# wolny/pytorch-3dunet

Hardware: AMD Instinct MI355X
Metric: volumetric patches/sec (fwd+bwd), UNet3D f_maps=32 patch 64x128x128 (higher is better)
Workload: dtype f32

## Files before the change

include/u3d.h:

```cpp
#ifndef U3D_H
#define U3D_H

#include <stddef.h>
#include <stdint.h>

#ifdef __cplusplus
extern "C" {
#endif

#define U3D_VERSION 128

#define U3D_OK 0
#define U3D_EINVAL (-1)
#define U3D_EHIP (-2)
#define U3D_EARCH (-3)
#define U3D_EWORKSPACE (-4)

typedef void* u3d_stream_t;

typedef struct {
    const float* p0;
    const float* p1;
    const int32_t* zmap;
    const int32_t* ymap;
    const int32_t* xmap;
    const float* affine;
    int32_t C0, C1;
    int32_t D1, H1, W1;
} u3d_src_t;

int u3d_version(void);
const char* u3d_last_error(void);
int u3d_check_device(int device);
int u3d_set_tuning(int key, int value);
int u3d_set_profile_buffer(void* device_buffer, size_t bytes);
int u3d_debug_stream_pass(int device, u3d_stream_t stream, float* buf, long long n, int blocks, int passes, double min_seconds);
int u3d_debug_mfma_f32_rate(int device, u3d_stream_t stream, float* sink, int iters, int mode, double* flop_out);

size_t u3d_packed_weight_floats(int Cin, int Cout, int mode);
int u3d_pack_weights(int device, u3d_stream_t stream, const float* w, int Cout, int Cin, int mode, float* packed);
typedef struct {
    const float* w;
    float* packed;
    int64_t first;
    int32_t Cout, Cin, mode, cin_stride;
} u3d_pack_desc_t;
int u3d_pack_weights_batch(int device, u3d_stream_t stream, const u3d_pack_desc_t* descs_device, int n,
                           int64_t total_floats);
long long u3d_pack_weights_cells_blocks(const float* w, int Cin, int Cout, int mode, int cin_stride);
int u3d_pack_weights_batch_cells(int device, u3d_stream_t stream, const u3d_pack_desc_t* descs_device, int n, long long total_blocks);

int u3d_conv3d(int device, u3d_stream_t stream, const u3d_src_t* src, const float* packed_w, float* out,
               int N, int D, int H, int W, int Cout, int relu, double* out_stats, const u3d_src_t* gx,
               double* gstats);

int u3d_conv3d_residual(int device, u3d_stream_t stream, const u3d_src_t* src, const float* packed_w, float* out,
                        int N, int D, int H, int W, int Cout, int relu, double* out_stats, const float* residual);

long long u3d_conv3d_workspace_floats(int N, int D, int H, int W, int Cin, int Cout);
int u3d_conv3d_ex(int device, u3d_stream_t stream, const u3d_src_t* src, const float* packed_w, float* out, int N,
                  int D, int H, int W, int Cout, int relu, double* out_stats, const u3d_src_t* gx, double* gstats,
                  const float* residual, float* workspace, long long workspace_floats);

int u3d_conv3d_ex_reps(int device, u3d_stream_t stream, const u3d_src_t* src, const float* packed_w, float* out, int N,
                       int D, int H, int W, int Cout, int relu, double* out_stats, const u3d_src_t* gx, double* gstats,
                       const float* residual, float* workspace, long long workspace_floats, int stat_reps);

long long u3d_subpixel_packed_floats(int C1, int Cout);
long long u3d_subpixel_dgrad_packed_floats(int Cout, int C1);
int u3d_pack_subpixel_dgrad_weights(int device, u3d_stream_t stream, const float* w, int Cout, int Cin_total, int c_off,
                                    int C1, float* packed);
int u3d_subpixel_conv_dgrad(int device, u3d_stream_t stream, const float* dz, const float* packed, const float* x_low,
                            float* dlow, double* gstats, int N, int D1, int H1, int W1, int C1, int Cout);
int u3d_subpixel_conv_dgrad_reps(int device, u3d_stream_t stream, const float* dz, const float* packed, const float* x_low, float* dlow,
                                 double* gstats, int N, int D1, int H1, int W1, int C1, int Cout, int reps);
int u3d_pack_subpixel_weights(int device, u3d_stream_t stream, const float* w, int Cout, int Cin_total, int c_off, int C1,
                              float* packed);
long long u3d_subpixel_fwd_workspace_floats(int N, int D1, int H1, int W1, int C1, int Cout);
int u3d_subpixel_conv_fwd(int device, u3d_stream_t stream, const float* low, const float* affine,
                          long long affine_sample_stride, const float* packed, float* out, int N, int D1, int H1, int W1,
                          int C1, int Cout, float* workspace, long long workspace_floats);

size_t u3d_wgrad_workspace_floats(int N, int D, int H, int W, int Cin, int Cout);
int u3d_conv3d_wgrad(int device, u3d_stream_t stream, const u3d_src_t* src, const float* dz, float* dw, int N,
                     int D, int H, int W, int Cout, float* workspace, size_t workspace_floats);

int u3d_conv3d_variant(int N, int D, int H, int W, int Cin, int Cout, int src_kind, int has_workspace);
int u3d_conv3d_wgrad_variant(int N, int D, int H, int W, int Cin, int Cout, int src_kind);

int u3d_conv3d_wgrad_strided(int device, u3d_stream_t stream, const u3d_src_t* src, const float* dz, float* dw,
                             int dw_cin_stride, int N, int D, int H, int W, int Cout, float* workspace,
                             size_t workspace_floats);

typedef struct u3d_gn_bwd_job {
    const double* gstats_lo;
    const double* gstats_hi;
    const float* mean_rstd;
    const float* gamma;
    float* dgamma;
    float* dbeta;
    float* coef;
    float* coef_hi;
    double count;
    int32_t C0, C1, N, G;
    float hi_scale;
    int32_t reps_lo;
    int32_t reps_hi;
    int32_t reserved;
} u3d_gn_bwd_job_t;
int u3d_conv3d_wgrad_job_supported(int N, int C, int G);
int u3d_conv3d_wgrad_job(int device, u3d_stream_t stream, const u3d_src_t* src, const float* dz, float* dw, int dw_cin_stride,
                         int N, int D, int H, int W, int Cout, float* workspace, size_t workspace_floats,
                         const u3d_gn_bwd_job_t* job);

long long u3d_subpixel_wgrad_workspace_floats(int N, int D1, int H1, int W1, int C1, int Cout);
int u3d_subpixel_conv_wgrad(int device, u3d_stream_t stream, const float* low, const float* affine,
                            long long affine_sample_stride, const float* dz, float* dw, int dw_cin_stride, int N, int D1,
                            int H1, int W1, int C1, int Cout, float* workspace, long long workspace_floats);

int u3d_subpixel_conv_fwd_win(int device, u3d_stream_t stream, const float* low, const float* affine, long long affine_sample_stride,
                              const float* packed, float* out, int N, int D1, int H1, int W1, int C1, int Cout, const int* win);
int u3d_subpixel_conv_dgrad_win(int device, u3d_stream_t stream, const float* dz, const float* packed, const float* x_low, float* dlow,
                                double* gstats, int N, int D1, int H1, int W1, int C1, int Cout, const int* win);
int u3d_subpixel_conv_wgrad_win(int device, u3d_stream_t stream, const float* low, const float* affine, long long affine_sample_stride,
                                const float* dz, float* dw, int dw_cin_stride, int N, int D1, int H1, int W1, int C1, int Cout,
                                float* workspace, long long workspace_floats, const int* win);
int u3d_conv3d_box(int device, u3d_stream_t stream, const u3d_src_t* src, const float* packed_w, float* out, int N, int D, int H, int W,
                   int Cout, const int* out_box, const int* in_mask);
int u3d_conv3d_wgrad_box(int device, u3d_stream_t stream, const u3d_src_t* src, const float* dz, float* dw, int N, int D, int H, int W,
                         int Cout, float* workspace, size_t workspace_floats, const int* box);
int u3d_gn_bwd_apply_children(int device, u3d_stream_t stream, const float* dlow, const float* x, const float* coef, int Ctot, int coff,
                              int N, int D1, int H1, int W1, int C, int ez, int ey, int ex, int relu_mask, float* out);
int u3d_chan_stats_children(int device, u3d_stream_t stream, const float* x_low, int N, int D1, int H1, int W1, int C, int ez, int ey,
                            int ex, double* stats);
int u3d_nearest_childsum_add(int device, u3d_stream_t stream, const float* dv, const float* x_low, float* dlow, double* gstats, int N,
                             int D, int H, int W, int D1, int H1, int W1, int C, const int32_t* zlo, const int32_t* ylo,
                             const int32_t* xlo, int cz, int cy, int cx);

int u3d_conv3d_small_cin_fwd(int device, u3d_stream_t stream, const float* x, const float* affine, const float* w,
                             float* out, int N, int D, int H, int W, int Cin, int Cout, int relu, double* out_stats);
int u3d_conv3d_small_cin_fwd_reps(int device, u3d_stream_t stream, const float* x, const float* affine, const float* w, float* out, int N,
                                  int D, int H, int W, int Cin, int Cout, int relu, double* out_stats, int reps);
size_t u3d_small_cin_bwd_workspace_floats(int N, int D, int H, int W, int Cin, int Cout);
int u3d_conv3d_small_cin_bwd(int device, u3d_stream_t stream, const float* x, const float* affine, const float* dz,
                             const float* w, float* dw, double* gstats, int N, int D, int H, int W, int Cin, int Cout,
                             float* workspace, size_t workspace_floats);

int u3d_conv3d_naive(int device, u3d_stream_t stream, const u3d_src_t* src, const float* w, float* out, int N,
                     int D, int H, int W, int Cin, int Cout, int relu, int flip);
// ... 313 lines not shown
```

pytorch-3dunet_amd/csrc/u3d_conv.hip:

```cpp
#include <type_traits>
#include <utility>

#include "u3d_common.h"
#include "u3d_gn.h"
#include "u3d_subpix.h"

int g_u3d_tune[24] = {0};

namespace cv {
constexpr int TZ = 4, TY = 8, TX = 8;
constexpr int HZ = TZ + 2, HY = TY + 2, HX = TX + 2;
constexpr int CC = 16;
constexpr int CS = 16;
constexpr int RS = HX * CS + 4;
constexpr int PS = HY * RS;
constexpr int TILE_FLOATS = HZ * PS + 4;
constexpr int CNT_OFF = 2 * TILE_FLOATS;
constexpr int RED_OFF = CNT_OFF + 16;
constexpr int LDS_FLOATS = RED_OFF + 4 * 3 * 32 * 2;
constexpr int NITEMS = HZ * HY * HX * (CC / 4);
constexpr int NIT = (NITEMS + 255) / 256;
constexpr int NSTEP = 27 * (CC / 8);
constexpr int NSTEP_PAIRY = 36 * (CC / 8);
constexpr int NSTEP_N16 = 27;
constexpr int ST0 = 30;
constexpr int ISTORE = 5;
constexpr int PACK_PAD = 5;
static_assert(2 * (NIT - 1) < ST0 - 8 && ST0 + NIT <= NSTEP, "prefetch schedule must fit the k-loop");
}

struct ConvParams {
    u3d_src_t src;
    u3d_src_t gx;
    const float* wp;
    float* out;
    double* out_stats;
    double* gstats;
    const float* res;
    int N, D, H, W, Cout;
    int nchunks, ncb, ntot;
    int tz, ty, tx;
    int relu, vec, has_gx, ovec;
    int total;
    int gx_x2;
    int stagger;
    int stat_reps;
    int zfast;
    int ksplit, cps;
    long long part_stride;
    long long* dbg;
    int oz0, oy0, ox0, oz1, oy1, ox1;
    int mz, my, mx;
};

#define U3D_DBG_STAMP(slot)                                                   \
    do {                                                                      \
        if constexpr (DBG) {                                                  \
            if (l == 0) dbgw[slot] = (long long)__builtin_readcyclecounter(); \
        }                                                                     \
    } while (0)

__device__ __forceinline__ void u3d_flag_signal(int* c, int lane) {
    asm volatile("" ::: "memory");
    if (lane == 0) __hip_atomic_fetch_add(c, 1, __ATOMIC_RELAXED, __HIP_MEMORY_SCOPE_WORKGROUP);
    asm volatile("" ::: "memory");
}
__device__ __forceinline__ void u3d_flag_wait(int* c, int target) {
    while (__hip_atomic_load(c, __ATOMIC_RELAXED, __HIP_MEMORY_SCOPE_WORKGROUP) < target) __builtin_amdgcn_s_sleep(2);
    asm volatile("" ::: "memory");
}

template <int NT, bool VEC, bool DBG = false, int ABL = 0>
__global__ __launch_bounds__(256, 2) void conv3d_mfma_kernel(const ConvParams p) {
    using namespace cv;
    constexpr int RB = NT == 1 ? 6 : 3;
    extern __shared__ __attribute__((aligned(16))) float lds[];
    int* cnt = reinterpret_cast<int*>(lds + CNT_OFF);
    const int t = threadIdx.x;
    const int l = t & 63, w = t >> 6, m = l & 31, h = l >> 5;
    __builtin_amdgcn_s_setprio(3);
    long long* dbgw = nullptr;
    if constexpr (DBG) {
        dbgw = p.dbg + ((size_t)blockIdx.x * 4 + w) * 24;
        if (l == 0) {
            dbgw[0] = blockIdx.x;
            dbgw[1] = __builtin_amdgcn_s_getreg((31 << 11) | 4);
            dbgw[2] = __builtin_amdgcn_s_getreg((31 << 11) | 20);
            dbgw[7] = p.nchunks;
        }
    }
    U3D_DBG_STAMP(3);
    if (t < 16) cnt[t] = 0;
    __syncthreads();

    int logical = u3d_xcd_remap(blockIdx.x, gridDim.x);
    int ch0 = 0, nch = p.nchunks;
    float* const outp = p.out + (size_t)(p.ksplit > 1 ? logical % p.ksplit : 0) * p.part_stride;
    if (p.ksplit > 1) {
        ch0 = (logical % p.ksplit) * p.cps;
        nch = min(p.cps, p.nchunks - ch0);
        logical /= p.ksplit;
    }
    const int cb = logical % p.ncb;
    int tile = logical / p.ncb;
    const int txi = tile % p.tx;
    tile /= p.tx;
    const int tyi = tile % p.ty;
    tile /= p.ty;
    const int tzi = tile % p.tz;
    const int n = tile / p.tz;
    const int z0 = p.oz0 + tzi * TZ, y0 = p.oy0 + tyi * TY, x0 = p.ox0 + txi * TX;
    const int D = p.D, H = p.H, W = p.W;
    const int Ctot = p.src.C0 + p.src.C1;
    const bool slab_mask = (p.mz | p.my | p.mx) != 0;

    int ldsoff[NIT], gv0[NIT], gv1[NIT];
    const int q = t & 3;
#pragma unroll
    for (int it = 0; it < NIT; ++it) {
        const int item = t + 256 * it;
        const int vox = item >> 2;
        const bool in = item < NITEMS;
        const int hz = vox / (HY * HX);
        const int rem = vox - hz * (HY * HX);
        const int hy = rem / HX;
        const int hx = rem - hy * HX;
        ldsoff[it] = in ? hz * PS + hy * RS + hx * CS + 4 * q : HZ * PS;
        const int gz = z0 - 1 + hz, gy = y0 - 1 + hy, gxx = x0 - 1 + hx;
        bool ok = in && gz >= 0 && gz < D && gy >= 0 && gy < H && gxx >= 0 && gxx < W;
        if (slab_mask) ok = ok && ((p.mz && gz < p.mz) || (p.my && gy < p.my) || (p.mx && gxx < p.mx));
        gv0[it] = -1;
        gv1[it] = 0;
        if (ok) u3d_vox_index(p.src, n, gz, gy, gxx, D, H, W, gv0[it], gv1[it]);
    }

// ... 313 lines not shown
        if (arrived == 3) {
            for (int k = l; k < NT * 32; k += 64) {
                const int nt = k >> 5, mm = k & 31;
                float a = 0.f, b = 0.f;
#pragma unroll
                for (int ww = 0; ww < 4; ++ww) {
                    a += red[((ww * NT + nt) * 32 + mm) * 2 + 0];
                    b += red[((ww * NT + nt) * 32 + mm) * 2 + 1];
                }
                const int co = (cb * NT + nt) * 32 + mm;
                if (co < p.Cout) {
                    double* dst = (want_stats ? p.out_stats : p.gstats) + ((size_t)n * p.Cout + co) * 2;
                    u3d_atomic_add_f64(dst, (double)a);
                    u3d_atomic_add_f64(dst + 1, (double)b);
                }
            }
        }
    }
    U3D_DBG_STAMP(6);
}

struct SplitKParams {
    const float* part;
    long long stride;
    float* out;
    const float* res;
    double* stats;
    u3d_src_t gx;
    int ksplit, relu, want_g, V, D, H, W, C;
};

__global__ __launch_bounds__(256) void splitk_reduce_kernel(const SplitKParams p) {
    __shared__ double red[256 * 4 * 2];
    const int Q = p.C >> 2, per = blockDim.x / Q;
    const int t = threadIdx.x, cq = t % Q, vl = t / Q, n = blockIdx.y;
    for (int k = t; k < Q * 8; k += blockDim.x) red[k] = 0.0;
    __syncthreads();
    f32x4 s1 = {0.f, 0.f, 0.f, 0.f}, s2 = {0.f, 0.f, 0.f, 0.f};
    const bool xfrom0 = 4 * cq < p.gx.C0;
    for (int v = blockIdx.x * per + vl; v < p.V; v += gridDim.x * per) {
        const size_t off = ((size_t)n * p.V + v) * p.C + 4 * cq;
        f32x4 a = *reinterpret_cast<const f32x4*>(p.part + off);
        for (int k = 1; k < p.ksplit; ++k) a += *reinterpret_cast<const f32x4*>(p.part + (size_t)k * p.stride + off);
        if (p.res) a += *reinterpret_cast<const f32x4*>(p.res + off);
        if (p.relu) {
#pragma unroll
            for (int e = 0; e < 4; ++e) a[e] = fmaxf(a[e], 0.f);
        }
        *reinterpret_cast<f32x4*>(p.out + off) = a;
        if (p.stats) {
            s1 += a;
            if (p.want_g) {
                const int x = v % p.W, y = (v / p.W) % p.H, z = v / (p.W * p.H);
                int v0, v1;
                u3d_vox_index(p.gx, n, z, y, x, p.D, p.H, p.W, v0, v1);
                const f32x4 xv = xfrom0 ? *reinterpret_cast<const f32x4*>(p.gx.p0 + (size_t)v0 * p.gx.C0 + 4 * cq)
                                        : *reinterpret_cast<const f32x4*>(p.gx.p1 + (size_t)v1 * p.gx.C1 + (4 * cq - p.gx.C0));
                s2 += a * xv;
            } else {
                s2 += a * a;
            }
        }
    }
    if (p.stats) {
#pragma unroll
        for (int e = 0; e < 4; ++e) {
            __hip_atomic_fetch_add(&red[(cq * 4 + e) * 2], (double)s1[e], __ATOMIC_RELAXED, __HIP_MEMORY_SCOPE_WORKGROUP);
            __hip_atomic_fetch_add(&red[(cq * 4 + e) * 2 + 1], (double)s2[e], __ATOMIC_RELAXED, __HIP_MEMORY_SCOPE_WORKGROUP);
        }
        __syncthreads();
        for (int k = t; k < p.C * 2; k += blockDim.x) u3d_atomic_add_f64(&p.stats[(size_t)n * p.C * 2 + k], red[k]);
    }
}

template <int B, int... I, class F>
__device__ __forceinline__ void u3d_for_rows_impl(std::integer_sequence<int, I...>, F&& f) {
    (f(std::integral_constant<int, B + I>{}), ...);
}
template <int B, int E, class F>
__device__ __forceinline__ void u3d_for_rows(F&& f) {
    if constexpr (E > B) u3d_for_rows_impl<B>(std::make_integer_sequence<int, E - B>{}, static_cast<F&&>(f));
}

template <int NT, bool VIRT, bool DBG = false, bool PAIRY = false, bool AFF = true, bool N16 = false, bool RAG = false>
__global__ __launch_bounds__(256, 2) void conv3d_mfma_reg_kernel(const ConvParams p) {
    using namespace cv;
    static_assert(!RAG || (!PAIRY && !DBG), "ragged tiles: standard and 16-column variants only");
    static_assert(!PAIRY || NT == 1, "the paired-y variant has a single N-tile");
    static_assert(!N16 || (NT == 1 && !PAIRY), "the 16-column variant has a single N-tile");
    constexpr int RB = NT == 1 ? 9 : 3;
    constexpr int MT = N16 ? 4 : (PAIRY ? 1 : 2);
    constexpr int RY = PAIRY ? 4 : 3;
    constexpr int NROWS = 3 * RY;
    constexpr int SPR = N16 ? 3 : 6;
    constexpr int NSTEPL = NROWS * SPR;
    constexpr int DBG_TILE = 1;
    extern __shared__ __attribute__((aligned(16))) float lds[];
    int* cnt = reinterpret_cast<int*>(lds + CNT_OFF);
    double* red = reinterpret_cast<double*>(lds + RED_OFF);
    static_assert((RED_OFF * 4) % 8 == 0 && 2 * 3 * 32 * 2 * 8 <= 4 * 3 * 32 * 2 * 4, "f64 statistics rows must fit");
    const int t = threadIdx.x;
    const int l = t & 63, w = __builtin_amdgcn_readfirstlane(t >> 6), m = l & 31, h = l >> 5;
    __builtin_amdgcn_s_setprio(3);
    long long* dbgw = nullptr;
    if constexpr (DBG) {
        dbgw = p.dbg + ((size_t)blockIdx.x * 4 + w) * 24;
        if (l == 0) {
            dbgw[0] = blockIdx.x;
            dbgw[1] = __builtin_amdgcn_s_getreg((31 << 11) | 4);
            dbgw[2] = __builtin_amdgcn_s_getreg((31 << 11) | 20);
            dbgw[7] = p.nchunks;
        }
    }
    U3D_DBG_STAMP(3);
    if (t < 16) cnt[t] = 0;
    for (int k = t; k < 2 * 3 * 32 * 2; k += 256) red[k] = 0.0;
    __syncthreads();

    const int D = p.D, H = p.H, W = p.W;
    const int Ctot = p.src.C0 + p.src.C1;
    const int G = gridDim.x;
    const int D1 = p.src.D1, H1 = p.src.H1, W1 = p.src.W1;

    struct Item {
        int cb, n, z0, y0, x0;
        int base0, base1;
        unsigned inv;
        bool border;
    };
    const int q = t & 3, tv = t >> 2;
    int rel0[NIT], rel1[VIRT ? NIT : 1], loff[NIT];
    unsigned fz0 = 0, fz1 = 0, fy0 = 0, fy1 = 0, fx0 = 0, fx1 = 0, fdead = 0;
    const int vz = RAG && D % TZ ? D % TZ : TZ, vy = RAG && H % TY ? H % TY : TY, vx = RAG && W % TX ? W % TX : TX;
#pragma unroll
    for (int it = 0; it < NIT; ++it) {
        const int vox = tv + 64 * it;
        const bool in = vox < HZ * HY * HX;
        const int hz = vox / (HY * HX);
        const int rem = vox - hz * (HY * HX);
        const int hy = rem / HX;
        const int hx = rem - hy * HX;
        rel0[it] = in ? (hz * H + hy) * W + hx : 0;
        if constexpr (VIRT) rel1[it] = in ? (((hz - 1) >> 1) * H1 + ((hy - 1) >> 1)) * W1 + ((hx - 1) >> 1) : 0;
        loff[it] = in ? hz * PS + hy * RS + hx * CS + 4 * q : HZ * PS;
        fz0 |= (in && hz == 0 ? 1u : 0u) << it;
        fz1 |= (in && hz > vz ? 1u : 0u) << it;
        fy0 |= (in && hy == 0 ? 1u : 0u) << it;
        fy1 |= (in && hy > vy ? 1u : 0u) << it;
        fx0 |= (in && hx == 0 ? 1u : 0u) << it;
        fx1 |= (in && hx > vx ? 1u : 0u) << it;
        fdead |= (in ? 0u : 1u) << it;
    }
    struct Digits {
        int cb, xi, yi, zi, n;
    };
    const bool zfast = p.zfast != 0;
    const int r1 = zfast ? p.tz : p.tx, r3 = zfast ? p.tx : p.tz;
    auto decode = [&](int idx) {
        Digits d;
        d.cb = idx % p.ncb;
        int tile = idx / p.ncb;
        d.xi = tile % r1;
        tile /= r1;
        d.yi = tile % p.ty;
        tile /= p.ty;
        d.zi = tile % r3;
        d.n = tile / r3;
        return d;
    };
    const Digits dG = decode(G);
    auto advance = [&](const Digits& a) {
        Digits r;
        int c;
        r.cb = a.cb + dG.cb;
        c = r.cb >= p.ncb ? 1 : 0;
        r.cb -= c ? p.ncb : 0;
        r.xi = a.xi + dG.xi + c;
        c = r.xi >= r1 ? 1 : 0;
        r.xi -= c ? r1 : 0;
        r.yi = a.yi + dG.yi + c;
        c = r.yi >= p.ty ? 1 : 0;
        r.yi -= c ? p.ty : 0;
        r.zi = a.zi + dG.zi + c;
        c = r.zi >= r3 ? 1 : 0;
        r.zi -= c ? r3 : 0;
        r.n = a.n + dG.n + c;
        return r;
    };
    auto item_of = [&](const Digits& d) {
        Item c;
        c.cb = d.cb;
        c.x0 = (zfast ? d.zi : d.xi) * TX;
        c.y0 = d.yi * TY;
        c.z0 = (zfast ? d.xi : d.zi) * TZ;
        c.n = d.n;
        c.base0 = ((c.n * D + c.z0 - 1) * H + c.y0 - 1) * W + c.x0 - 1;
        c.base1 = VIRT ? ((c.n * D1 + (c.z0 >> 1)) * H1 + (c.y0 >> 1)) * W1 + (c.x0 >> 1) : 0;
        const bool bz0 = c.z0 == 0, bz1 = c.z0 + TZ >= D, by0 = c.y0 == 0, by1 = c.y0 + TY >= H, bx0 = c.x0 == 0,
                   bx1 = c.x0 + TX >= W;
        c.border = bz0 || bz1 || by0 || by1 || bx0 || bx1;
        c.inv = fdead | (bz0 ? fz0 : 0u) | (bz1 ? fz1 : 0u) | (by0 ? fy0 : 0u) | (by1 ? fy1 : 0u) | (bx0 ? fx0 : 0u) |
                (bx1 ? fx1 : 0u);
        return c;
    };
    int wi = u3d_xcd_remap(blockIdx.x, G);
    Digits dT = decode(wi);
    Item T = item_of(dT);

    constexpr bool ZEROC = NT < 3 && !N16;
    f32x16 acc[N16 ? 1 : MT][NT];
    f32x4 acc16[N16 ? MT : 1];
    if constexpr (N16) {
#pragma unroll
        for (int mt = 0; mt < MT; ++mt) acc16[mt] = f32x4{0.f, 0.f, 0.f, 0.f};
    } else if constexpr (!ZEROC) {
#pragma unroll
        for (int mt = 0; mt < MT; ++mt)
#pragma unroll
            for (int nt = 0; nt < NT; ++nt)
#pragma unroll
                for (int r = 0; r < 16; ++r) acc[mt][nt][r] = 0.f;
    }

    const int v16 = l & 15, kq = l >> 4;
    const int abase = N16 ? w * PS + 2 * (v16 >> 3) * RS + (v16 & 7) * CS + 4 * kq
                          : w * PS + (m >> 3) * (PAIRY ? 2 : 1) * RS + (m & 7) * CS + 4 * h;
    auto mrow = [](int mt) { return N16 ? (mt >> 1) * 4 + (mt & 1) : 4 * mt; };

    const f32x4* wimg = reinterpret_cast<const f32x4*>(p.wp);
    const f32x4* wq = wimg + (size_t)T.cb * NT * 64;
    const int wstep = p.ntot * 64;
    f32x4 bq[RB][NT];
#pragma unroll
    for (int k = 0; k < RB - 1; ++k)
#pragma unroll
        for (int nt = 0; nt < NT; ++nt) bq[k][nt] = wq[(size_t)k * wstep + nt * 64 + l];

    struct ChunkSrc {
        const float* base;
        int Cs;
        bool cok, from0;
        const float* ap;
        f32x4 lo, hi;
    };
    auto chunk_src = [&](int ch, int n, bool live) {
        ChunkSrc c;
        const int cq = ch * CC + 4 * q;
        c.cok = live && cq < Ctot;
        c.from0 = !VIRT || cq < p.src.C0;
        c.base = !c.cok ? p.src.p0 : (c.from0 ? p.src.p0 + cq : p.src.p1 + (cq - p.src.C0));
        c.Cs = (c.from0 || !c.cok) ? p.src.C0 : p.src.C1;
        c.ap = p.src.affine ? p.src.affine + ((size_t)n * Ctot + (c.cok ? cq : 0)) * 2 : nullptr;
        c.lo = f32x4{1.f, 0.f, 1.f, 0.f};
        c.hi = f32x4{1.f, 0.f, 1.f, 0.f};
        return c;
    };
    auto load_affine_rows = [&](ChunkSrc& c) {
        if constexpr (AFF) {
            if (c.ap) {
                c.lo = *reinterpret_cast<const f32x4*>(c.ap);
                c.hi = *reinterpret_cast<const f32x4*>(c.ap + 4);
            }
        }
    };
    auto halo_load = [&](const ChunkSrc& c, const Item& S, int it, bool masked) {
        int idx = c.from0 ? S.base0 + rel0[it] : S.base1 + rel1[VIRT ? it : 0];
        if (masked) idx = (c.cok && ((S.inv >> it) & 1u) == 0) ? idx : 0;
        return *reinterpret_cast<const f32x4*>(c.base + (size_t)idx * c.Cs);
    };
    auto halo_store = [&](float* buf, const ChunkSrc& c, const Item& S, int it, f32x4 raw, bool masked) {
        f32x4 val = raw;
        if constexpr (AFF)
            val = f32x4{fmaf(raw[0], c.lo[0], c.lo[1]), fmaf(raw[1], c.lo[2], c.lo[3]), fmaf(raw[2], c.hi[0], c.hi[1]),
                        fmaf(raw[3], c.hi[2], c.hi[3])};
        if (masked) {
            const bool ok = c.cok && ((S.inv >> it) & 1u) == 0;
#pragma unroll
            for (int e = 0; e < 4; ++e) val[e] = ok ? val[e] : 0.f;
        }
        *reinterpret_cast<f32x4*>(&buf[loff[it]]) = val;
    };
    const bool want_stats = p.out_stats != nullptr;
    const bool want_g = p.gstats != nullptr;
    auto flush_stats = [&](int n, int cb) {
        if (!(want_stats || want_g)) return;
        const int par = n & 1;
        int arrived = 0;
        asm volatile("" ::: "memory");
        if (l == 0) arrived = __hip_atomic_fetch_add(&cnt[5 + par], 1, __ATOMIC_RELAXED, __HIP_MEMORY_SCOPE_WORKGROUP);
        arrived = __builtin_amdgcn_readfirstlane(arrived);
        asm volatile("" ::: "memory");
        if ((arrived & 3) != 3) return;
        const int rep = p.stat_reps > 1 ? (int)(blockIdx.x % (unsigned)p.stat_reps) : 0;
        for (int k = l; k < NT * 32; k += 64) {
            double* r = &red[(par * NT * 32 + k) * 2];
            const double a = r[0], b = r[1];
            r[0] = 0.0;
            r[1] = 0.0;
            const int co = cb * NT * 32 + k;
            if (co < p.Cout) {
                double* dst = (want_stats ? p.out_stats : p.gstats) + ((size_t)rep * p.N * p.Cout + (size_t)n * p.Cout + co) * 2;
                u3d_atomic_add_f64(dst, a);
                u3d_atomic_add_f64(dst + 1, b);
            }
        }
        asm volatile("" ::: "memory");
    };
    const bool dead_quads = (Ctot % CC) != 0;

    {
        ChunkSrc c0 = chunk_src(0, T.n, true);
        load_affine_rows(c0);
        const bool masked = T.border || dead_quads || fdead != 0;
        f32x4 v[NIT];
#pragma unroll
        for (int it = 0; it < NIT; ++it) v[it] = halo_load(c0, T, it, true);
#pragma unroll
        for (int it = 0; it < NIT; ++it) halo_store(lds, c0, T, it, v[it], true);
        (void)masked;
    }
    u3d_flag_signal(&cnt[0], l);

    if (p.stagger > 0 && (int)blockIdx.x >= (G + 1) / 2) {
        for (int i = 0; i < p.stagger; ++i) __builtin_amdgcn_s_sleep(16);
    }

    int gch = 0;
    int ntiles = 0;
    constexpr bool CARRY = NT == 1;
    f32x4 sq1 = {0.f, 0.f, 0.f, 0.f}, sq2 = {0.f, 0.f, 0.f, 0.f};
    auto quad_sum = [](float v) {
        v += __builtin_bit_cast(float, __builtin_amdgcn_mov_dpp(__builtin_bit_cast(int, v), 0xB1, 0xF, 0xF, true));
        v += __builtin_bit_cast(float, __builtin_amdgcn_mov_dpp(__builtin_bit_cast(int, v), 0x4E, 0xF, 0xF, true));
        return v;
    };
    auto stat_reduce = [&](const f32x4& a1, const f32x4& a2, int n_, int nt_, int c0) {
#pragma unroll
        for (int e = 0; e < 4; ++e) {
            const float a = quad_sum(a1[e]), b2 = quad_sum(a2[e]);
            if ((l & 3) == 0) {
                double* r = &red[(((n_ & 1) * NT + nt_) * 32 + c0 + e) * 2];
                __hip_atomic_fetch_add(r, (double)a, __ATOMIC_RELAXED, __HIP_MEMORY_SCOPE_WORKGROUP);
                __hip_atomic_fetch_add(r + 1, (double)b2, __ATOMIC_RELAXED, __HIP_MEMORY_SCOPE_WORKGROUP);
            }
        }
    };
    while (true) {
        const int nwi = wi + G;
        const bool has_next_tile = nwi < p.total;
        const Digits dTN = has_next_tile ? advance(dT) : dT;
        const Item TN = item_of(dTN);
        const f32x4* wqn = wimg + (size_t)TN.cb * NT * 64;

        for (int ch = 0; ch < p.nchunks; ++ch, ++gch) {
            const bool last = ch + 1 == p.nchunks;
            const bool has_next = !last || has_next_tile;
            const int b = gch & 1;
            const float* cur = lds + b * TILE_FLOATS;
            float* nxt = lds + (b ^ 1) * TILE_FLOATS;
            const int nch_ = last ? 0 : ch + 1;
            const Item S = last ? TN : T;
            ChunkSrc cn = chunk_src(nch_, S.n, has_next);
            const bool masked = S.border || !has_next || (dead_quads && nch_ + 1 == p.nchunks);
            f32x4 v[NIT];
            u3d_flag_wait(&cnt[b], 4 * (gch / 2 + 1));
            __builtin_amdgcn_s_setprio(0);
            if (ntiles == DBG_TILE && ch < 7) U3D_DBG_STAMP(8 + 2 * ch);
            if (ntiles == DBG_TILE + 1 && ch == 0) U3D_DBG_STAMP(23);

            f32x4 aq[2][MT];
#pragma unroll
            for (int mt = 0; mt < MT; ++mt) aq[0][mt] = *reinterpret_cast<const f32x4*>(&cur[abase + mrow(mt) * RS]);
            const f32x4* wch0 = wq + (size_t)(ch * NSTEPL + RB - 1) * wstep;
            enum { ROW_PLAIN = 0, ROW_LOAD = 1, ROW_AFFINE = 2, ROW_STORE = 3, ROW_LAST = 4, ROW_LOAD_FIRST = 5 };
            auto row_body = [&](auto kind_c, auto row_c) __attribute__((always_inline)) {
                constexpr int KIND = decltype(kind_c)::value;
                constexpr int row = decltype(row_c)::value;
                const int rz = row / RY, ry = row - RY * rz;
                const float* arow = cur + abase + rz * PS + ry * RS;
                const int nrow = row + 1;
                const float* anext = cur + abase + (nrow / RY) * PS + (nrow % RY) * RS;
                const bool do_store = KIND == ROW_STORE && has_next;
                if constexpr (KIND == ROW_AFFINE) load_affine_rows(cn);
                if constexpr (KIND == ROW_STORE) {
                    if (do_store) u3d_flag_wait(&cnt[2 + (b ^ 1)], 4 * ((gch + 1) / 2));
                }
#pragma unroll
                for (int s6 = 0; s6 < SPR; ++s6) {
                    constexpr int STORES_PER_STEP = (NIT + SPR - 2) / (SPR - 1);
                    {
                        const f32x4* wsrc = wch0 + (size_t)(row * SPR + s6) * wstep;
                        if (row * SPR + s6 + RB - 1 >= NSTEPL && last) wsrc = wqn + (size_t)(row * SPR + s6 + RB - 1 - NSTEPL) * wstep;
#pragma unroll
                        for (int nt = 0; nt < NT; ++nt) bq[(row * SPR + s6 + RB - 1) % RB][nt] = wsrc[nt * 64 + l];
                    }
                    if constexpr (KIND == ROW_LOAD || KIND == ROW_LOAD_FIRST) {
                        if (s6 == 0) {
                            if (masked) {
#pragma unroll
                                for (int it = 0; it < NIT; ++it) v[it] = halo_load(cn, S, it, true);
                            } else {
#pragma unroll
                                for (int it = 0; it < NIT; ++it) v[it] = halo_load(cn, S, it, false);
                            }
                        }
                    }
                    __builtin_amdgcn_sched_barrier(0);
#pragma unroll
                    for (int j = 0; j < 2; ++j) {
                        if constexpr (N16) {
#pragma unroll
                            for (int mt = 0; mt < MT; ++mt)
                                acc16[mt] = __builtin_amdgcn_mfma_f32_16x16x4f32(bq[(row * SPR + s6) % RB][0][j], aq[(row * SPR + s6) & 1][mt][j], acc16[mt], 0, 0, 0);
                        } else {
#pragma unroll
                            for (int nt = 0; nt < NT; ++nt) {
#pragma unroll
                                for (int mt = 0; mt < MT; ++mt) {
                                    if (KIND == ROW_LOAD_FIRST && s6 == 0 && j == 0) {
                                        const f32x16 zero = {0.f, 0.f, 0.f, 0.f, 0.f, 0.f, 0.f, 0.f, 0.f, 0.f, 0.f, 0.f, 0.f, 0.f, 0.f, 0.f};
                                        acc[mt][nt] = __builtin_amdgcn_mfma_f32_32x32x2f32(aq[0][mt][0], bq[0][nt][0], zero, 0, 0, 0);
                                    } else {
                                        acc[mt][nt] = __builtin_amdgcn_mfma_f32_32x32x2f32(aq[(row * SPR + s6) & 1][mt][j], bq[(row * SPR + s6) % RB][nt][j], acc[mt][nt], 0, 0, 0);
                                    }
                                }
                            }
                        }
                    }
                    __builtin_amdgcn_sched_barrier(0);
                    if (s6 < SPR - 1) {
                        const int aoff = N16 ? (s6 + 1) * CS : ((s6 + 1) >> 1) * CS + 8 * ((s6 + 1) & 1);
#pragma unroll
                        for (int mt = 0; mt < MT; ++mt) aq[(row * SPR + s6 + 1) & 1][mt] = *reinterpret_cast<const f32x4*>(&arow[mrow(mt) * RS + aoff]);
                    } else if constexpr (KIND != ROW_LAST) {
#pragma unroll
                        for (int mt = 0; mt < MT; ++mt) aq[(row * SPR + s6 + 1) & 1][mt] = *reinterpret_cast<const f32x4*>(&anext[mrow(mt) * RS]);
                    }
                    if constexpr (KIND == ROW_STORE) {
                        if (do_store && s6 * STORES_PER_STEP < NIT) {
#pragma unroll
                            for (int k = 0; k < STORES_PER_STEP; ++k) {
                                const int it = s6 * STORES_PER_STEP + k;
                                if (it < NIT) {
                                    if (masked)
                                        halo_store(nxt, cn, S, it, v[it], true);
                                    else
                                        halo_store(nxt, cn, S, it, v[it], false);
                                }
                            }
                            if ((s6 + 1) * STORES_PER_STEP >= NIT) u3d_flag_signal(&cnt[b ^ 1], l);
                        }
                    }
                    __builtin_amdgcn_sched_barrier(0);
#pragma unroll
                    for (int j = 2; j < 4; ++j) {
                        if constexpr (N16) {
#pragma unroll
                            for (int mt = 0; mt < MT; ++mt)
                                acc16[mt] = __builtin_amdgcn_mfma_f32_16x16x4f32(bq[(row * SPR + s6) % RB][0][j], aq[(row * SPR + s6) & 1][mt][j], acc16[mt], 0, 0, 0);
                        } else {
#pragma unroll
                            for (int nt = 0; nt < NT; ++nt) {
#pragma unroll
                                for (int mt = 0; mt < MT; ++mt)
                                    acc[mt][nt] = __builtin_amdgcn_mfma_f32_32x32x2f32(aq[(row * SPR + s6) & 1][mt][j], bq[(row * SPR + s6) % RB][nt][j], acc[mt][nt], 0, 0, 0);
                            }
                        }
                    }
                    __builtin_amdgcn_sched_barrier(0);
                }
            };
            static_assert(ISTORE - 1 > 1 && ISTORE + 1 < NROWS - 1, "row kinds must not collide");
            static_assert(NSTEPL % RB == 0, "B ring slots are indexed by the k-step within the chunk");
            using R0 = std::integral_constant<int, 0>;
            if (ZEROC && ch == 0)
                row_body(std::integral_constant<int, ROW_LOAD_FIRST>{}, R0{});
            else
                row_body(std::integral_constant<int, ROW_LOAD>{}, R0{});
            u3d_for_rows<1, ISTORE - 1>([&](auto r) { row_body(std::integral_constant<int, ROW_PLAIN>{}, r); });
            row_body(std::integral_constant<int, ROW_AFFINE>{}, std::integral_constant<int, ISTORE - 1>{});
            row_body(std::integral_constant<int, ROW_STORE>{}, std::integral_constant<int, ISTORE>{});
            u3d_for_rows<ISTORE + 1, NROWS - 1>([&](auto r) { row_body(std::integral_constant<int, ROW_PLAIN>{}, r); });
            row_body(std::integral_constant<int, ROW_LAST>{}, std::integral_constant<int, NROWS - 1>{});
            if (ntiles == DBG_TILE && ch < 7) U3D_DBG_STAMP(9 + 2 * ch);
            u3d_flag_signal(&cnt[2 + b], l);
        }
        __builtin_amdgcn_s_setprio(3);

        if (ntiles == DBG_TILE) U3D_DBG_STAMP(5);
        if constexpr (N16) {
            const int n = T.n;
            const int z = T.z0 + w;
            const int co = 4 * kq;
            const bool cok = co < p.Cout;
            const int vlane = ((n * D + z) * H + T.y0 + 2 * (v16 >> 3)) * W + T.x0 + (v16 & 7);
            float* orow = p.out + (size_t)vlane * p.Cout + co;
            const size_t rstep = (size_t)W * p.Cout;
            auto vin = [&](int mt) { return !RAG || (z < D && T.y0 + mrow(mt) + 2 * (v16 >> 3) < H && T.x0 + (v16 & 7) < W); };
            f32x4 xv[MT];
            if (want_g) {
                const bool from0 = co < p.gx.C0 || !cok;
#pragma unroll
                for (int mt = 0; mt < MT; ++mt) {
                    const int y = T.y0 + mrow(mt) + 2 * (v16 >> 3), x = T.x0 + (v16 & 7);
                    const int xi1 = ((n * p.gx.D1 + (z >> 1)) * p.gx.H1 + (y >> 1)) * p.gx.W1 + (x >> 1);
                    const float* xp = !(cok && vin(mt)) ? p.gx.p0
                                           : (from0 ? p.gx.p0 + (size_t)(vlane + mrow(mt) * W) * p.gx.C0 + co
                                                    : p.gx.p1 + (size_t)xi1 * p.gx.C1 + (co - p.gx.C0));
                    xv[mt] = *reinterpret_cast<const f32x4*>(xp);
                }
            } else if (p.res) {
#pragma unroll
                for (int mt = 0; mt < MT; ++mt)
                    xv[mt] = *reinterpret_cast<const f32x4*>(p.res + (vin(mt) ? (size_t)(vlane + mrow(mt) * W) * p.Cout + (cok ? co : 0) : (size_t)0));
            }
#pragma unroll
            for (int mt = 0; mt < MT; ++mt) {
                f32x4 val = acc16[mt];
                if (p.res) val += xv[mt];
                if (p.relu) {
#pragma unroll
                    for (int e = 0; e < 4; ++e) val[e] = fmaxf(val[e], 0.f);
                }
                if (cok && vin(mt)) *reinterpret_cast<f32x4*>(orow + mrow(mt) * rstep) = val;
                if (RAG || p.Cout % 16 != 0) {
#pragma unroll
                    for (int e = 0; e < 4; ++e) val[e] = (cok && vin(mt)) ? val[e] : 0.f;
                }
                sq1 += val;
                sq2 += want_g ? val * xv[mt] : val * val;
                acc16[mt] = f32x4{0.f, 0.f, 0.f, 0.f};
            }
        } else
        if (p.stagger != -1) {
            const int n = T.n, cb = T.cb;
            const int z = T.z0 + w;
            const int cq = (l >> 2) & 7, vl = (l & 3) + 4 * h;
            const bool odd = (l & 1) != 0, hi = (l & 2) != 0;
            auto xlane = [](float v, auto ctrl) {
                return __builtin_bit_cast(float, __builtin_amdgcn_mov_dpp(__builtin_bit_cast(int, v), decltype(ctrl)::value, 0xF, 0xF, true));
            };
            using X1 = std::integral_constant<int, 0xB1>;
            using X2 = std::integral_constant<int, 0x4E>;
            const int vrow = ((n * D + z) * H + T.y0) * W + T.x0 + vl;
            const int xrow = ((n * p.gx.D1 + (z >> 1)) * p.gx.H1 + (T.y0 >> 1)) * p.gx.W1 + ((T.x0 + vl) >> 1);
#pragma unroll
            for (int nt = 0; nt < NT; ++nt) {
                f32x4 q1 = {0.f, 0.f, 0.f, 0.f}, q2 = {0.f, 0.f, 0.f, 0.f};
                f32x4 tq[4 * MT];
#pragma unroll
                for (int mt = 0; mt < MT; ++mt)
#pragma unroll
                    for (int bi = 0; bi < 4; ++bi) {
                        const float a0 = acc[mt][nt][4 * bi + 0], a1 = acc[mt][nt][4 * bi + 1];
                        const float a2 = acc[mt][nt][4 * bi + 2], a3 = acc[mt][nt][4 * bi + 3];
                        const float t0 = xlane(a1, X1{}), t1 = xlane(a0, X1{}), t2 = xlane(a3, X1{}), t3 = xlane(a2, X1{});
                        const float c0 = odd ? t0 : a0, c1 = odd ? a1 : t1, c2 = odd ? t2 : a2, c3 = odd ? a3 : t3;
                        const float u0 = xlane(c2, X2{}), u2 = xlane(c0, X2{}), u1 = xlane(c3, X2{}), u3 = xlane(c1, X2{});
                        tq[4 * mt + bi] = f32x4{hi ? u0 : c0, hi ? u1 : c1, hi ? c2 : u2, hi ? c3 : u3};
                    }
                const int ysh = PAIRY ? (cq >> 2) : 0;
                const int co = PAIRY ? 4 * (cq & 3) : (cb * NT + nt) * 32 + 4 * cq;
// ... 793 lines not shown
            const int f = fq * (sp::NFRAG / PK_SUBQ) + (i >> 6), lane = i & 63;
            const int st = sp::frag_tab().st[f];
            const int kl = 8 * (st & 1) + 4 * (lane >> 5), nl = lane & 31;
            f32x4 v;
#pragma unroll
            for (int j = 0; j < 4; ++j) v[j] = sp::frag_value(row_of(nl, kl + j), f);
            out4[(((long long)ch * sp::NFRAG + f) * ntot + ntg) * 64 + lane] = v;
        }
    } else {
        for (int i = t; i < spd::NFRAG / PK_SUBQ * 64; i += 256) {
            const int f = fq * (spd::NFRAG / PK_SUBQ) + (i >> 6), lane = i & 63;
            const int kl = 8 * (f & 1) + 4 * (lane >> 5), nl = lane & 31;
            f32x4 v;
#pragma unroll
            for (int j = 0; j < 4; ++j) v[j] = spd::frag_value(row_of(nl, kl + j), f);
            out4[(((long long)ch * spd::NFRAG + f) * ntot + ntg) * 64 + lane] = v;
        }
    }
}

__global__ void conv3d_naive_kernel(const u3d_src_t src, const float* __restrict__ w, float* __restrict__ out,
                                    int N, int D, int H, int W, int Cin, int Cout, int relu, int flip) {
    const long long total = (long long)N * D * H * W * Cout;
    for (long long idx = (long long)blockIdx.x * blockDim.x + threadIdx.x; idx < total;
         idx += (long long)gridDim.x * blockDim.x) {
        const int co = (int)(idx % Cout);
        long long v = idx / Cout;
        const int x = (int)(v % W);
        v /= W;
        const int y = (int)(v % H);
        v /= H;
        const int z = (int)(v % D);
        const int n = (int)(v / D);
        float sum = 0.f;
        for (int tap = 0; tap < 27; ++tap) {
            const int zz = z + tap / 9 - 1, yy = y + (tap / 3) % 3 - 1, xx = x + tap % 3 - 1;
            if (zz < 0 || zz >= D || yy < 0 || yy >= H || xx < 0 || xx >= W) continue;
            int v0, v1;
            u3d_vox_index(src, n, zz, yy, xx, D, H, W, v0, v1);
            for (int c = 0; c < Cin; ++c) {
                float g = u3d_load_elem(src, v0, v1, c);
                if (src.affine) {
                    const float* ab = src.affine + ((size_t)n * Cin + c) * 2;
                    g = g * ab[0] + ab[1];
                }
                const float wt = flip ? w[((size_t)c * Cout + co) * 27 + (26 - tap)] : w[((size_t)co * Cin + c) * 27 + tap];
                sum += g * wt;
            }
        }
        if (relu) sum = fmaxf(sum, 0.f);
        out[idx] = sum;
    }
}

static inline int cdiv(int a, int b) { return (a + b - 1) / b; }

static bool src_vec_ok(const u3d_src_t* s) {
    if (s->C0 % 4 != 0 || s->C1 % 4 != 0) return false;
    if (((uintptr_t)s->p0 & 15) != 0) return false;
    if (s->C1 > 0 && ((uintptr_t)s->p1 & 15) != 0) return false;
    if (s->affine && ((uintptr_t)s->affine & 15) != 0) return false;
    return true;
}

static int check_src(const u3d_src_t* s, const char* what) {
    U3D_REQUIRE(s != nullptr && s->p0 != nullptr && (s->C0 > 0 || s->C1 > 0) && s->C0 >= 0, "%s: null source", what);
    U3D_REQUIRE(s->C1 >= 0, "%s: negative C1", what);
    if (s->C1 > 0)
        U3D_REQUIRE(s->p1 && s->zmap && s->ymap && s->xmap && s->D1 > 0 && s->H1 > 0 && s->W1 > 0,
                    "%s: low-res source needs p1, index maps and dims", what);
    return 0;
}

static long long* g_u3d_prof_buf = nullptr;
static size_t g_u3d_prof_records = 0;

extern "C" int u3d_set_profile_buffer(void* device_buffer, size_t bytes) {
    g_u3d_prof_buf = static_cast<long long*>(device_buffer);
    g_u3d_prof_records = device_buffer ? bytes / (24 * sizeof(long long)) : 0;
    return 0;
}

extern "C" int u3d_set_tuning(int key, int value) {
    if (key < 0 || key >= 24) return u3d_set_err(U3D_EINVAL, "u3d_set_tuning: key out of range");
    g_u3d_tune[key] = value;
    return 0;
}

extern "C" size_t u3d_packed_weight_floats(int Cin, int Cout, int mode) {
    return (size_t)pack_total_floats(Cin, Cout, mode, nullptr, nullptr);
}

extern "C" int u3d_pack_weights(int device, u3d_stream_t stream, const float* w, int Cout, int Cin, int mode,
                                float* packed) {
    U3D_ENTER(device);
    U3D_REQUIRE(w && packed && Cout > 0 && Cin > 0 && (mode == 0 || mode == 1), "u3d_pack_weights: bad argument");
    int nchunks = 0, ntot = 0;
    const long long total = pack_total_floats(Cin, Cout, mode, &nchunks, &ntot);
    const int blocks = (int)((total + 255) / 256 > 4096 ? 4096 : (total + 255) / 256);
    hipLaunchKernelGGL(pack_weights_kernel, dim3(blocks), dim3(256), 0, (hipStream_t)stream, w, packed, Cout, Cin,
                       mode, nchunks, ntot, total);
    U3D_LAUNCH_CHECK();
    return 0;
}

extern "C" int u3d_pack_weights_batch(int device, u3d_stream_t stream, const u3d_pack_desc_t* descs_device, int n,
                                      int64_t total_floats) {
    U3D_ENTER(device);
    U3D_REQUIRE(descs_device && n > 0 && total_floats > 0, "u3d_pack_weights_batch: bad argument");
    U3D_REQUIRE(total_floats % 4 == 0, "u3d_pack_weights_batch: image sizes are multiples of 4 floats");
    long long blocks = (total_floats / 4 + 255) / 256;
    if (blocks > 8192) blocks = 8192;
    hipLaunchKernelGGL(pack_weights_batch_kernel, dim3((unsigned)blocks), dim3(256), 0, (hipStream_t)stream, descs_device, n,
                       (long long)total_floats);
    U3D_LAUNCH_CHECK();
    return 0;
}

extern "C" long long u3d_pack_weights_cells_blocks(const float* w, int Cin, int Cout, int mode, int cin_stride) {
    const int cs = cin_stride > 0 ? cin_stride : Cin;
    if (Cin <= 0 || Cout <= 0 || mode < 0 || mode > 3 || Cin % 4 != 0 || Cout % 4 != 0 || cs % 4 != 0 || ((uintptr_t)w & 15) != 0) return 0;
    return pack_cells_of(Cin, Cout, mode) + 1;
}

extern "C" int u3d_pack_weights_batch_cells(int device, u3d_stream_t stream, const u3d_pack_desc_t* descs_device, int n,
                                            long long total_blocks) {
    U3D_ENTER(device);
    U3D_REQUIRE(descs_device && n > 0 && total_blocks > 0 && total_blocks < 0x7fffffffLL, "u3d_pack_weights_batch_cells: bad argument");
    hipLaunchKernelGGL(pack_weights_cells_kernel, dim3((unsigned)total_blocks), dim3(256), 0, (hipStream_t)stream, descs_device, n);
    U3D_LAUNCH_CHECK();
    return 0;
}

static int device_cu_count(int device, int* out) {
    static int cached[64] = {0};
    if (device >= 0 && device < 64 && cached[device] > 0) {
        *out = cached[device];
        return 0;
    }
    int n = 0;
    U3D_HIP(hipDeviceGetAttribute(&n, hipDeviceAttributeMultiprocessorCount, device));
    if (n <= 0) n = 256;
    if (device >= 0 && device < 64) cached[device] = n;
    *out = n;
    return 0;
}

template <int NT>
static int conv_set_lds_nt() {
    const int bytes = cv::LDS_FLOATS * sizeof(float);
    U3D_HIP(hipFuncSetAttribute(reinterpret_cast<const void*>(conv3d_mfma_reg_kernel<NT, false, false>),
                                hipFuncAttributeMaxDynamicSharedMemorySize, bytes));
    U3D_HIP(hipFuncSetAttribute(reinterpret_cast<const void*>(conv3d_mfma_reg_kernel<NT, true, false>),
                                hipFuncAttributeMaxDynamicSharedMemorySize, bytes));
    U3D_HIP(hipFuncSetAttribute(reinterpret_cast<const void*>(conv3d_mfma_reg_kernel<NT, false, true>),
                                hipFuncAttributeMaxDynamicSharedMemorySize, bytes));
    U3D_HIP(hipFuncSetAttribute(reinterpret_cast<const void*>(conv3d_mfma_reg_kernel<NT, true, true>),
                                hipFuncAttributeMaxDynamicSharedMemorySize, bytes));
    U3D_HIP(hipFuncSetAttribute(reinterpret_cast<const void*>(conv3d_mfma_reg_kernel<NT, false, false, false, false>),
                                hipFuncAttributeMaxDynamicSharedMemorySize, bytes));
    U3D_HIP(hipFuncSetAttribute(reinterpret_cast<const void*>(conv3d_mfma_reg_kernel<NT, true, false, false, true, false, true>),
                                hipFuncAttributeMaxDynamicSharedMemorySize, bytes));
    U3D_HIP(hipFuncSetAttribute(reinterpret_cast<const void*>(conv3d_mfma_reg_kernel<NT, false, false, false, false, false, true>),
                                hipFuncAttributeMaxDynamicSharedMemorySize, bytes));
    U3D_HIP(hipFuncSetAttribute(reinterpret_cast<const void*>(conv3d_mfma_reg_kernel<NT, false, false, false, true, false, true>),
                                hipFuncAttributeMaxDynamicSharedMemorySize, bytes));
    if (NT == 1) {
        U3D_HIP(hipFuncSetAttribute(reinterpret_cast<const void*>(conv3d_mfma_reg_kernel<1, true, false, false, true, true, true>),
                                    hipFuncAttributeMaxDynamicSharedMemorySize, bytes));
        U3D_HIP(hipFuncSetAttribute(reinterpret_cast<const void*>(conv3d_mfma_reg_kernel<1, false, false, false, false, true, true>),
                                    hipFuncAttributeMaxDynamicSharedMemorySize, bytes));
        U3D_HIP(hipFuncSetAttribute(reinterpret_cast<const void*>(conv3d_mfma_reg_kernel<1, false, false, false, true, true, true>),
                                    hipFuncAttributeMaxDynamicSharedMemorySize, bytes));
        U3D_HIP(hipFuncSetAttribute(reinterpret_cast<const void*>(conv3d_mfma_reg_kernel<1, false, false, true, false>),
                                    hipFuncAttributeMaxDynamicSharedMemorySize, bytes));
        U3D_HIP(hipFuncSetAttribute(reinterpret_cast<const void*>(conv3d_mfma_reg_kernel<1, false, false, true>),
                                    hipFuncAttributeMaxDynamicSharedMemorySize, bytes));
        U3D_HIP(hipFuncSetAttribute(reinterpret_cast<const void*>(conv3d_mfma_reg_kernel<1, true, false, true>),
                                    hipFuncAttributeMaxDynamicSharedMemorySize, bytes));
        U3D_HIP(hipFuncSetAttribute(reinterpret_cast<const void*>(conv3d_mfma_reg_kernel<1, true, false, false, true, true>),
                                    hipFuncAttributeMaxDynamicSharedMemorySize, bytes));
        U3D_HIP(hipFuncSetAttribute(reinterpret_cast<const void*>(conv3d_mfma_reg_kernel<1, false, false, false, false, true>),
                                    hipFuncAttributeMaxDynamicSharedMemorySize, bytes));
        U3D_HIP(hipFuncSetAttribute(reinterpret_cast<const void*>(conv3d_mfma_reg_kernel<1, false, false, false, true, true>),
                                    hipFuncAttributeMaxDynamicSharedMemorySize, bytes));
    }
    U3D_HIP(hipFuncSetAttribute(reinterpret_cast<const void*>(conv3d_mfma_kernel<NT, true, false>),
                                hipFuncAttributeMaxDynamicSharedMemorySize, bytes));
    U3D_HIP(hipFuncSetAttribute(reinterpret_cast<const void*>(conv3d_mfma_kernel<NT, false, false>),
                                hipFuncAttributeMaxDynamicSharedMemorySize, bytes));
    U3D_HIP(hipFuncSetAttribute(reinterpret_cast<const void*>(conv3d_mfma_kernel<NT, true, true>),
                                hipFuncAttributeMaxDynamicSharedMemorySize, bytes));
    if (NT == 1) {
        U3D_HIP(hipFuncSetAttribute(reinterpret_cast<const void*>(conv3d_mfma_kernel<1, true, true, 1>),
                                    hipFuncAttributeMaxDynamicSharedMemorySize, bytes));
        U3D_HIP(hipFuncSetAttribute(reinterpret_cast<const void*>(conv3d_mfma_kernel<1, true, true, 2>),
                                    hipFuncAttributeMaxDynamicSharedMemorySize, bytes));
        U3D_HIP(hipFuncSetAttribute(reinterpret_cast<const void*>(conv3d_mfma_kernel<1, true, true, 3>),
                                    hipFuncAttributeMaxDynamicSharedMemorySize, bytes));
        U3D_HIP(hipFuncSetAttribute(reinterpret_cast<const void*>(conv3d_mfma_kernel<1, true, true, 7>),
                                    hipFuncAttributeMaxDynamicSharedMemorySize, bytes));
    }
    return 0;
}

static int conv_set_lds_once(int device) {
    static bool done[64] = {false};
    if (device >= 0 && device < 64 && done[device]) return 0;
    if (int e = conv_set_lds_nt<1>()) return e;
    if (int e = conv_set_lds_nt<2>()) return e;
    if (int e = conv_set_lds_nt<3>()) return e;
    if (device >= 0 && device < 64) done[device] = true;
    return 0;
}

static int conv3d_impl(int device, u3d_stream_t stream, const u3d_src_t* src, const float* packed_w, float* out, int N,
                       int D, int H, int W, int Cout, int relu, double* out_stats, const u3d_src_t* gx, double* gstats,
                       const float* residual, float* ws = nullptr, long long ws_floats = 0, const int* out_box = nullptr,
                       const int* in_mask = nullptr, int stat_reps = 1);

extern "C" int u3d_conv3d(int device, u3d_stream_t stream, const u3d_src_t* src, const float* packed_w, float* out,
                          int N, int D, int H, int W, int Cout, int relu, double* out_stats, const u3d_src_t* gx,
                          double* gstats) {
    return conv3d_impl(device, stream, src, packed_w, out, N, D, H, W, Cout, relu, out_stats, gx, gstats, nullptr);
}

extern "C" int u3d_conv3d_box(int device, u3d_stream_t stream, const u3d_src_t* src, const float* packed_w, float* out, int N, int D,
                              int H, int W, int Cout, const int* out_box, const int* in_mask) {
    return conv3d_impl(device, stream, src, packed_w, out, N, D, H, W, Cout, 0, nullptr, nullptr, nullptr, nullptr, nullptr, 0, out_box,
                       in_mask);
}

constexpr int SPLITK_MAX = 16;
static int g_u3d_ncu_seen = 256;
static int splitk_count(int ncu, long long ntiles, int ntot, int nchunks, int* cps_out) {
    long long ks = (2ll * ncu) / (ntiles * ntot);
    if (ks > nchunks) ks = nchunks;
    if (ks > SPLITK_MAX) ks = SPLITK_MAX;
    int cps = nchunks, ksplit = 1;
    if (ks >= 2) {
        cps = (nchunks + (int)ks - 1) / (int)ks;
        ksplit = (nchunks + cps - 1) / cps;
    }
    if (cps_out) *cps_out = cps;
    return ksplit;
}

static bool splitk_shape(int N, int D, int H, int W, int Cin, int Cout) {
    const long long items = (long long)N * cdiv(D, cv::TZ) * cdiv(H, cv::TY) * cdiv(W, cv::TX) * cdiv(Cout, 32);
    return Cin > 16 && Cout % 4 == 0 && Cout <= 1024 && items < 256;
}

extern "C" long long u3d_conv3d_workspace_floats(int N, int D, int H, int W, int Cin, int Cout) {
    if (N <= 0 || D <= 0 || H <= 0 || W <= 0 || Cin <= 0 || Cout <= 0 || !splitk_shape(N, D, H, W, Cin, Cout)) return 0;
    const int ks = cdiv(Cin, 16) < SPLITK_MAX ? cdiv(Cin, 16) : SPLITK_MAX;
    return (long long)ks * N * D * H * W * Cout;
}

extern "C" int u3d_conv3d_ex(int device, u3d_stream_t stream, const u3d_src_t* src, const float* packed_w, float* out,
                             int N, int D, int H, int W, int Cout, int relu, double* out_stats, const u3d_src_t* gx,
                             double* gstats, const float* residual, float* workspace, long long workspace_floats) {
    U3D_REQUIRE(!(residual && gx), "u3d_conv3d_ex: residual and gx are mutually exclusive");
    return conv3d_impl(device, stream, src, packed_w, out, N, D, H, W, Cout, relu, out_stats, gx, gstats, residual,
                       workspace, workspace_floats);
}

extern "C" int u3d_conv3d_ex_reps(int device, u3d_stream_t stream, const u3d_src_t* src, const float* packed_w, float* out,
                                  int N, int D, int H, int W, int Cout, int relu, double* out_stats, const u3d_src_t* gx,
                                  double* gstats, const float* residual, float* workspace, long long workspace_floats, int stat_reps) {
    U3D_REQUIRE(!(residual && gx), "u3d_conv3d_ex_reps: residual and gx are mutually exclusive");
    return conv3d_impl(device, stream, src, packed_w, out, N, D, H, W, Cout, relu, out_stats, gx, gstats, residual,
                       workspace, workspace_floats, nullptr, nullptr, stat_reps);
}

extern "C" int u3d_conv3d_residual(int device, u3d_stream_t stream, const u3d_src_t* src, const float* packed_w,
                                   float* out, int N, int D, int H, int W, int Cout, int relu, double* out_stats,
                                   const float* residual) {
    if (residual == nullptr) return u3d_set_err(U3D_EINVAL, "u3d_conv3d_residual: residual is NULL");
    return conv3d_impl(device, stream, src, packed_w, out, N, D, H, W, Cout, relu, out_stats, nullptr, nullptr, residual);
}

static int conv3d_impl(int device, u3d_stream_t stream, const u3d_src_t* src, const float* packed_w, float* out, int N,
                       int D, int H, int W, int Cout, int relu, double* out_stats, const u3d_src_t* gx, double* gstats,
                       const float* residual, float* ws, long long ws_floats, const int* out_box, const int* in_mask, int stat_reps) {
    U3D_ENTER(device);
    if (int e = check_src(src, "u3d_conv3d")) return e;
    U3D_REQUIRE(stat_reps >= 1 && stat_reps <= 64, "u3d_conv3d: stat_reps must be 1 .. 64");
    U3D_REQUIRE(packed_w && out && N > 0 && D > 0 && H > 0 && W > 0 && Cout > 0, "u3d_conv3d: bad argument");
    U3D_REQUIRE((long long)N * D * H * W < (1ll << 31), "u3d_conv3d: N*D*H*W must be < 2^31");
    U3D_REQUIRE(!(out_stats && gstats), "u3d_conv3d: out_stats and gstats are mutually exclusive");
    U3D_REQUIRE((gstats == nullptr) == (gx == nullptr), "u3d_conv3d: gx and gstats go together");
    U3D_REQUIRE(((uintptr_t)packed_w & 15) == 0, "u3d_conv3d: packed weights must be 16-byte aligned");
    ConvParams p;
    p.src = *src;
    if (gx) {
        if (int e = check_src(gx, "u3d_conv3d(gx)")) return e;
        U3D_REQUIRE(gx->C0 + gx->C1 == Cout, "u3d_conv3d: gx must have Cout channels");
        p.gx = *gx;
    } else {
        p.gx = *src;
    }
    p.has_gx = gx != nullptr;
    p.wp = packed_w;
    p.out = out;
    p.out_stats = out_stats;
    p.gstats = gstats;
    p.res = residual;
    p.N = N, p.D = D, p.H = H, p.W = W, p.Cout = Cout;
    const int Cin = src->C0 + src->C1;
    p.nchunks = cdiv(Cin, 16);
    p.ntot = cdiv(Cout, 32);
    p.tz = cdiv(D, cv::TZ), p.ty = cdiv(H, cv::TY), p.tx = cdiv(W, cv::TX);
    p.oz0 = p.oy0 = p.ox0 = 0, p.oz1 = D, p.oy1 = H, p.ox1 = W;
    p.mz = p.my = p.mx = 0;
    const bool boxed = out_box != nullptr || in_mask != nullptr;
    if (out_box) {
        U3D_REQUIRE(out_box[0] >= 0 && out_box[1] >= 0 && out_box[2] >= 0 && out_box[3] <= D && out_box[4] <= H && out_box[5] <= W &&
                        out_box[0] < out_box[3] && out_box[1] < out_box[4] && out_box[2] < out_box[5],
                    "u3d_conv3d_box: output box outside the volume or empty");
        p.oz0 = out_box[0], p.oy0 = out_box[1], p.ox0 = out_box[2], p.oz1 = out_box[3], p.oy1 = out_box[4], p.ox1 = out_box[5];
        p.tz = cdiv(p.oz1 - p.oz0, cv::TZ), p.ty = cdiv(p.oy1 - p.oy0, cv::TY), p.tx = cdiv(p.ox1 - p.ox0, cv::TX);
    }
    if (in_mask) p.mz = in_mask[0], p.my = in_mask[1], p.mx = in_mask[2];
    p.relu = relu;
    p.vec = src_vec_ok(src) ? 1 : 0;
    p.ovec = (Cout % 4 == 0 && ((uintptr_t)out & 15) == 0 && (!gx || src_vec_ok(gx)) &&
              (!residual || ((uintptr_t)residual & 15) == 0)) ? 1 : 0;
    const long long ntiles = (long long)N * p.tz * p.ty * p.tx;
    int nt = 1;
    if (p.ntot % 3 == 0 && ntiles * (p.ntot / 3) >= 512) nt = 3;
    else if (p.ntot % 2 == 0 && ntiles * (p.ntot / 2) >= 512) nt = 2;
    if (g_u3d_tune[0] >= 1 && g_u3d_tune[0] <= 3 && p.ntot % g_u3d_tune[0] == 0) nt = g_u3d_tune[0];
    p.ncb = p.ntot / nt;
    const long long nblk = ntiles * p.ncb;
    U3D_REQUIRE(nblk < (1ll << 31), "u3d_conv3d: grid too large");
    const size_t shmem = cv::LDS_FLOATS * sizeof(float);
    if (int e = conv_set_lds_once(device)) return e;
    hipStream_t st = (hipStream_t)stream;
    p.ksplit = 1, p.cps = p.nchunks, p.part_stride = 0;
    if (!boxed && ws && p.vec && p.ovec && ((uintptr_t)ws & 15) == 0 && splitk_shape(N, D, H, W, Cin, Cout) && g_u3d_tune[7] != 2) {
        int ncu = 0;
        if (int e = device_cu_count(device, &ncu)) return e;
        g_u3d_ncu_seen = ncu;
        const long long items = ntiles * p.ntot, out_elems = (long long)N * D * H * W * Cout;
        p.ksplit = splitk_count(ncu, ntiles, p.ntot, p.nchunks, &p.cps);
        if (p.ksplit >= 2 && (long long)p.ksplit * out_elems <= ws_floats) {
            p.ncb = p.ntot;
            p.part_stride = out_elems;
            p.out = ws;
            p.out_stats = nullptr, p.gstats = nullptr, p.res = nullptr, p.relu = 0, p.has_gx = 0, p.dbg = nullptr;
            const dim3 kgrid((unsigned)(items * p.ksplit)), kblock(256);
            hipLaunchKernelGGL((conv3d_mfma_kernel<1, true>), kgrid, kblock, shmem, st, p);
            U3D_LAUNCH_CHECK();
            SplitKParams r;
            r.part = ws, r.stride = out_elems, r.out = out, r.res = residual;
            r.stats = out_stats ? out_stats : gstats;
            r.gx = gx ? *gx : *src;
            r.ksplit = p.ksplit, r.relu = relu, r.want_g = gstats != nullptr;
            r.V = D * H * W, r.D = D, r.H = H, r.W = W, r.C = Cout;
            const int Q = Cout / 4, per = 256 / Q;
            int gxb = cdiv(r.V, per * 4);
            const int cap = 256 / N > 1 ? 256 / N : 1;
            if (gxb > cap) gxb = cap;
            hipLaunchKernelGGL(splitk_reduce_kernel, dim3((unsigned)gxb, (unsigned)N), dim3((unsigned)(Q * per)), 0, st, r);
            U3D_LAUNCH_CHECK();
            return 0;
        }
        p.ksplit = 1, p.cps = p.nchunks;
    }
    auto plain_or_x2 = [&](const u3d_src_t& s_) {
        return s_.C1 == 0 || (D == 2 * s_.D1 && H == 2 * s_.H1 && W == 2 * s_.W1);
    };
    const bool ragged = D % cv::TZ != 0 || H % cv::TY != 0 || W % cv::TX != 0;
    const bool reg = p.vec && p.ovec && plain_or_x2(p.src) && (!gx || plain_or_x2(p.gx)) && g_u3d_tune[3] == 0 ||
                     (g_u3d_tune[3] == 2 && !ragged && p.vec && p.ovec && plain_or_x2(p.src) && (!gx || plain_or_x2(p.gx)));
    if (reg && !boxed) {
        p.total = (int)nblk;
        p.gx_x2 = (gx && p.gx.C1 > 0) ? 1 : 0;
        p.stagger = g_u3d_tune[5];
        p.stat_reps = stat_reps;
        p.zfast = g_u3d_tune[14] == 1 ? 0 : 1;
        int ncu = 0;
        if (int e = device_cu_count(device, &ncu)) return e;
        long long slots = (g_u3d_tune[6] == 1 ? 1ll : 2ll) * ncu;
        if (g_u3d_tune[12] > 0 && g_u3d_tune[12] < slots / 2) slots -= g_u3d_tune[12];
        if (slots >= nblk)
            slots = nblk;
        else if (slots > p.ncb)
            slots -= slots % p.ncb;
        const dim3 rgrid((unsigned)slots), rblock(256);
        const bool virt = p.src.C1 > 0;
        const bool noaff = p.src.affine == nullptr && g_u3d_tune[7] == 0;
        p.dbg = (!ragged && g_u3d_prof_buf && (size_t)slots * 4 <= g_u3d_prof_records) ? g_u3d_prof_buf : nullptr;
        if (ragged) {
            if (Cout <= 16 && nt == 1 && p.ntot == 1) {
                p.wp = packed_w + ((size_t)p.nchunks * cv::NSTEP + cv::PACK_PAD) * 256 + ((size_t)p.nchunks * cv::NSTEP_PAIRY + cv::PACK_PAD) * 256;
                if (virt)
                    hipLaunchKernelGGL((conv3d_mfma_reg_kernel<1, true, false, false, true, true, true>), rgrid, rblock, shmem, st, p);
                else if (noaff)
                    hipLaunchKernelGGL((conv3d_mfma_reg_kernel<1, false, false, false, false, true, true>), rgrid, rblock, shmem, st, p);
                else
                    hipLaunchKernelGGL((conv3d_mfma_reg_kernel<1, false, false, false, true, true, true>), rgrid, rblock, shmem, st, p);
                U3D_LAUNCH_CHECK();
                return 0;
            }
#define U3D_RAG_LAUNCH(NT_)                                                                                                        \
    do {                                                                                                                           \
        if (virt)                                                                                                                  \
            hipLaunchKernelGGL((conv3d_mfma_reg_kernel<NT_, true, false, false, true, false, true>), rgrid, rblock, shmem, st, p);  \
        else if (noaff)                                                                                                            \
            hipLaunchKernelGGL((conv3d_mfma_reg_kernel<NT_, false, false, false, false, false, true>), rgrid, rblock, shmem, st, p); \
        else                                                                                                                       \
            hipLaunchKernelGGL((conv3d_mfma_reg_kernel<NT_, false, false, false, true, false, true>), rgrid, rblock, shmem, st, p); \
    } while (0)
            if (nt == 3)
                U3D_RAG_LAUNCH(3);
            else if (nt == 2)
                U3D_RAG_LAUNCH(2);
            else
                U3D_RAG_LAUNCH(1);
#undef U3D_RAG_LAUNCH
            U3D_LAUNCH_CHECK();
            return 0;
        }
        if (Cout <= 16 && nt == 1 && p.ntot == 1 && !p.dbg && g_u3d_tune[4] != 1) {
            const size_t std_floats = ((size_t)p.nchunks * cv::NSTEP + cv::PACK_PAD) * 256;
            if (g_u3d_tune[4] == 2) {
                p.wp = packed_w + std_floats;
                if (virt)
                    hipLaunchKernelGGL((conv3d_mfma_reg_kernel<1, true, false, true>), rgrid, rblock, shmem, st, p);
                else if (noaff)
                    hipLaunchKernelGGL((conv3d_mfma_reg_kernel<1, false, false, true, false>), rgrid, rblock, shmem, st, p);
                else
                    hipLaunchKernelGGL((conv3d_mfma_reg_kernel<1, false, false, true>), rgrid, rblock, shmem, st, p);
            } else {
                p.wp = packed_w + std_floats + ((size_t)p.nchunks * cv::NSTEP_PAIRY + cv::PACK_PAD) * 256;
                if (virt)
                    hipLaunchKernelGGL((conv3d_mfma_reg_kernel<1, true, false, false, true, true>), rgrid, rblock, shmem, st, p);
                else if (noaff)
                    hipLaunchKernelGGL((conv3d_mfma_reg_kernel<1, false, false, false, false, true>), rgrid, rblock, shmem, st, p);
                else
                    hipLaunchKernelGGL((conv3d_mfma_reg_kernel<1, false, false, false, true, true>), rgrid, rblock, shmem, st, p);
            }
            U3D_LAUNCH_CHECK();
            return 0;
        }
#define U3D_REG_LAUNCH(NT_)                                                                                \
    do {                                                                                                   \
        if (p.dbg && virt)                                                                                 \
            hipLaunchKernelGGL((conv3d_mfma_reg_kernel<NT_, true, true>), rgrid, rblock, shmem, st, p);    \
        else if (p.dbg)                                                                                    \
            hipLaunchKernelGGL((conv3d_mfma_reg_kernel<NT_, false, true>), rgrid, rblock, shmem, st, p);   \
        else if (virt)                                                                                     \
            hipLaunchKernelGGL((conv3d_mfma_reg_kernel<NT_, true, false>), rgrid, rblock, shmem, st, p);   \
        else if (noaff)                                                                                    \
            hipLaunchKernelGGL((conv3d_mfma_reg_kernel<NT_, false, false, false, false>), rgrid, rblock,   \
                               shmem, st, p);                                                              \
        else                                                                                               \
            hipLaunchKernelGGL((conv3d_mfma_reg_kernel<NT_, false, false>), rgrid, rblock, shmem, st, p);  \
    } while (0)
        if (nt == 3)
            U3D_REG_LAUNCH(3);
        else if (nt == 2)
            U3D_REG_LAUNCH(2);
        else
            U3D_REG_LAUNCH(1);
#undef U3D_REG_LAUNCH
        U3D_LAUNCH_CHECK();
        return 0;
    }
    const bool vec = p.vec != 0;
    const dim3 grid((unsigned)nblk), block(256);
    p.dbg = (vec && g_u3d_prof_buf && (size_t)nblk * 4 <= g_u3d_prof_records) ? g_u3d_prof_buf : nullptr;
#define U3D_CONV_LAUNCH(NT_)                                                                     \
    do {                                                                                         \
        if (p.dbg && NT_ == 1 && g_u3d_tune[2] == 1)                                             \
            hipLaunchKernelGGL((conv3d_mfma_kernel<1, true, true, 1>), grid, block, shmem, st, p); \
        else if (p.dbg && NT_ == 1 && g_u3d_tune[2] == 2)                                        \
            hipLaunchKernelGGL((conv3d_mfma_kernel<1, true, true, 2>), grid, block, shmem, st, p); \
        else if (p.dbg && NT_ == 1 && g_u3d_tune[2] == 3)                                        \
            hipLaunchKernelGGL((conv3d_mfma_kernel<1, true, true, 3>), grid, block, shmem, st, p); \
        else if (p.dbg && NT_ == 1 && g_u3d_tune[2] == 7)                                        \
            hipLaunchKernelGGL((conv3d_mfma_kernel<1, true, true, 7>), grid, block, shmem, st, p); \
        else if (p.dbg)                                                                          \
            hipLaunchKernelGGL((conv3d_mfma_kernel<NT_, true, true>), grid, block, shmem, st, p); \
        else if (vec)                                                                            \
            hipLaunchKernelGGL((conv3d_mfma_kernel<NT_, true>), grid, block, shmem, st, p);      \
        else                                                                                     \
            hipLaunchKernelGGL((conv3d_mfma_kernel<NT_, false>), grid, block, shmem, st, p);     \
    } while (0)
    if (nt == 3)
        U3D_CONV_LAUNCH(3);
    else if (nt == 2)
        U3D_CONV_LAUNCH(2);
    else
        U3D_CONV_LAUNCH(1);
#undef U3D_CONV_LAUNCH
    U3D_LAUNCH_CHECK();
    return 0;
}

static void wgrad_plan(int N, int D, int H, int W, int Cin, int Cout, WgradParams& p) {
    p.nchunks = cdiv(Cin, 32);
    p.nkb = cdiv(Cout, 32);
    p.tz = cdiv(D, wg::TZ), p.ty = cdiv(H, wg::TY), p.tx = cdiv(W, wg::TX);
    p.ntiles = N * p.tz * p.ty * p.tx;
    const int pairs = p.nchunks * p.nkb;
    const int ncu = 256;
    long long best_cost = -1;
    int best_S = 1;
    for (int rounds = 1; rounds <= 8; ++rounds) {
        int S = (rounds * ncu) / pairs;
        if (S < 1) S = 1;
        if (S > p.ntiles) S = p.ntiles;
        const int tps = cdiv(p.ntiles, S);
        S = cdiv(p.ntiles, tps);
        const long long cost = (long long)cdiv(S * pairs, ncu) * (tps + 2);
        if (best_cost < 0 || cost < best_cost) {
            best_cost = cost;
            best_S = S;
        }
    }
    if (g_u3d_tune[1] > 0) best_S = g_u3d_tune[1] > p.ntiles ? p.ntiles : g_u3d_tune[1];
    p.tps = cdiv(p.ntiles, best_S);
    p.S = cdiv(p.ntiles, p.tps);
}

extern "C" size_t u3d_wgrad_workspace_floats(int N, int D, int H, int W, int Cin, int Cout) {
    WgradParams p;
    wgrad_plan(N, D, H, W, Cin, Cout, p);
    return (size_t)p.S * p.nchunks * p.nkb * 27 * 1024;
}

static int wgrad_set_lds_once(int device) {
    static bool done[64] = {false};
    if (device >= 0 && device < 64 && done[device]) return 0;
    U3D_HIP(hipFuncSetAttribute(reinterpret_cast<const void*>(conv3d_wgrad_kernel<true, true>),
                                hipFuncAttributeMaxDynamicSharedMemorySize, (wg::LDS_FLOATS + wg::MAX_MAP_INTS) * sizeof(float)));
    U3D_HIP(hipFuncSetAttribute(reinterpret_cast<const void*>(conv3d_wgrad_kernel<true, true, true>),
                                hipFuncAttributeMaxDynamicSharedMemorySize, (wg::LDS_FLOATS + wg::MAX_MAP_INTS) * sizeof(float)));
    U3D_HIP(hipFuncSetAttribute(reinterpret_cast<const void*>(conv3d_wgrad_kernel<true>),
                                hipFuncAttributeMaxDynamicSharedMemorySize, (wg::LDS_FLOATS + wg::MAX_MAP_INTS) * sizeof(float)));
    U3D_HIP(hipFuncSetAttribute(reinterpret_cast<const void*>(conv3d_wgrad_kernel<false>),
                                hipFuncAttributeMaxDynamicSharedMemorySize, (wg::LDS_FLOATS + wg::MAX_MAP_INTS) * sizeof(float)));
    if (device >= 0 && device < 64) done[device] = true;
    return 0;
}

static int conv3d_wgrad_impl(int device, u3d_stream_t stream, const u3d_src_t* src, const float* dz, float* dw, int cstride,
                             int N, int D, int H, int W, int Cout, float* workspace, size_t workspace_floats, const int* box = nullptr,
                             const u3d_gn_bwd_job_t* job = nullptr);

extern "C" int u3d_conv3d_wgrad_box(int device, u3d_stream_t stream, const u3d_src_t* src, const float* dz, float* dw, int N, int D,
// ... 135 lines not shown
```

pytorch-3dunet_amd/csrc/u3d_gn.h:

```cpp
#pragma once
#include "u3d_common.h"

__device__ __forceinline__ double u3d_sum_replicas(const double* __restrict__ p, size_t stride, int reps) {
    double v = p[0];
    for (int r0 = 1; r0 < reps; r0 += 8) {
        double t[8];
#pragma unroll
        for (int j = 0; j < 8; ++j) t[j] = r0 + j < reps ? p[(size_t)(r0 + j) * stride] : 0.0;
#pragma unroll
        for (int j = 0; j < 8; ++j) v += t[j];
    }
    return v;
}

__device__ inline void u3d_gn_bwd_finalize_body(const double* __restrict__ gs, const float* __restrict__ mean_rstd,
                                                const float* __restrict__ gamma, int N, int C, int G, double count, int staged, int par,
                                                float* __restrict__ dgamma, float* __restrict__ dbeta, float* __restrict__ coef,
                                                const double* __restrict__ gs_hi, int C0, float hi_scale, float* __restrict__ coef_hi,
                                                double* shb, int reps = 1, int reps_hi = 1) {

#pragma clang fp contract(off)
    const double* src = gs;
    if (staged) {
        if (gs_hi) {
            const int C1 = C - C0;
            for (int i = threadIdx.x; i < N * C * 2; i += blockDim.x) {
                const int e = i & 1, nc = i >> 1, n = nc / C, c = nc - n * C;
                shb[i] = c < C0 ? u3d_sum_replicas(gs + ((size_t)n * C0 + c) * 2 + e, (size_t)N * C0 * 2, reps)
                                : u3d_sum_replicas(gs_hi + ((size_t)n * C1 + (c - C0)) * 2 + e, (size_t)N * C1 * 2, reps_hi);
            }
        } else {
            for (int i = threadIdx.x; i < N * C * 2; i += blockDim.x) shb[i] = u3d_sum_replicas(gs + i, (size_t)N * C * 2, reps);
        }
        __syncthreads();
        src = shb;
    }
    const int cpg = C / G;
    const double m = count * cpg;
    double* pa = shb + 2 * (size_t)N * C;
    double* pb = pa + (size_t)N * C;
    double* qr = pb + (size_t)N * C;
    if (par) {
        for (int i = threadIdx.x; i < N * C; i += blockDim.x) {
            const int n = i / C, c = i - n * C, g = c / cpg;
            const double mean = (double)mean_rstd[((size_t)n * G + g) * 2], rstd = (double)mean_rstd[((size_t)n * G + g) * 2 + 1];
            const double S1 = src[(size_t)i * 2], S2 = src[(size_t)i * 2 + 1], gm = (double)gamma[c];
            pa[i] = gm * S1;
            pb[i] = gm * rstd * (S2 - mean * S1);
        }
        __syncthreads();
    }
    for (int pair = threadIdx.x; pair < N * G; pair += blockDim.x) {
        const int n = pair / G, g = pair - n * G;
        const double mean = (double)mean_rstd[(size_t)pair * 2], rstd = (double)mean_rstd[(size_t)pair * 2 + 1];
        double A = 0.0, B = 0.0;
        for (int c = g * cpg; c < (g + 1) * cpg; ++c) {
            if (par) {
                A += pa[(size_t)n * C + c];
                B += pb[(size_t)n * C + c];
            } else {
                const double S1 = src[((size_t)n * C + c) * 2], S2 = src[((size_t)n * C + c) * 2 + 1];
                const double gm = (double)gamma[c];
                A += gm * S1;
                B += gm * rstd * (S2 - mean * S1);
            }
        }
        const double q = -rstd * rstd * B / m;
        const double r = -rstd * A / m + rstd * rstd * mean * B / m;
        if (par) {
            qr[(size_t)pair * 2] = q;
            qr[(size_t)pair * 2 + 1] = r;
        } else {
            for (int c = g * cpg; c < (g + 1) * cpg; ++c) {
                coef[((size_t)n * 3 + 0) * C + c] = (float)(rstd * (double)gamma[c]);
                coef[((size_t)n * 3 + 1) * C + c] = (float)q;
                coef[((size_t)n * 3 + 2) * C + c] = (float)r;
            }
        }
    }
    if (par) {
        __syncthreads();
        for (int i = threadIdx.x; i < N * C; i += blockDim.x) {
            const int n = i / C, c = i - n * C, pair = n * G + c / cpg;
            const double rstd = (double)mean_rstd[(size_t)pair * 2 + 1];
            const float fp = (float)(rstd * (double)gamma[c]), fq = (float)qr[(size_t)pair * 2], fr = (float)qr[(size_t)pair * 2 + 1];
            coef[((size_t)n * 3 + 0) * C + c] = fp;
            coef[((size_t)n * 3 + 1) * C + c] = fq;
            coef[((size_t)n * 3 + 2) * C + c] = fr;
            if (coef_hi && c >= C0) {
                const int C1 = C - C0;
                coef_hi[((size_t)n * 3 + 0) * C1 + (c - C0)] = fp;
                coef_hi[((size_t)n * 3 + 1) * C1 + (c - C0)] = fq * hi_scale;
                coef_hi[((size_t)n * 3 + 2) * C1 + (c - C0)] = fr * hi_scale;
            }
        }
// ... 15 lines not shown
```

pytorch-3dunet_amd/csrc/u3d_ops.hip:

```cpp
#include "u3d_common.h"
#include "u3d_gn.h"

#include <string.h>

extern int g_u3d_tune[24];

static thread_local char g_err[512] = "";

int u3d_set_err(int code, const char* fmt, ...) {
    va_list ap;
    va_start(ap, fmt);
    vsnprintf(g_err, sizeof(g_err), fmt, ap);
    va_end(ap);
    return code;
}

int u3d_device_guard::enter(int device) {
    hipError_t e = hipGetDevice(&prev);
    if (e != hipSuccess) return u3d_set_err(U3D_EHIP, "hipGetDevice failed: %s", hipGetErrorString(e));
    if (device >= 0 && prev != device) {
        e = hipSetDevice(device);
        if (e != hipSuccess) return u3d_set_err(U3D_EHIP, "hipSetDevice(%d) failed: %s", device, hipGetErrorString(e));
        switched = true;
    }
// ... 388 lines not shown
}

extern "C" int u3d_gn_finalize_split(int device, u3d_stream_t stream, const double* stats0, int C0, double scale0,
                                     const double* stats1, int C1, double scale1, int N, int G, double count,
                                     const float* gamma, const float* beta, float eps, float* affine, float* mean_rstd,
                                     int Csplit, float* affine_lo, float* affine_hi) {
    return gn_finalize_impl(device, stream, stats0, C0, scale0, stats1, C1, scale1, N, G, count, gamma, beta, eps, affine, mean_rstd,
                            affine_lo, affine_hi, Csplit);
}

extern "C" int u3d_gn_finalize_reps(int device, u3d_stream_t stream, const double* stats0, int C0, double scale0, int reps0,
                                    const double* stats1, int C1, double scale1, int reps1, int N, int G, double count,
                                    const float* gamma, const float* beta, float eps, float* affine, float* mean_rstd,
                                    int Csplit, float* affine_lo, float* affine_hi) {
    return gn_finalize_impl(device, stream, stats0, C0, scale0, stats1, C1, scale1, N, G, count, gamma, beta, eps, affine, mean_rstd,
                            affine_lo, affine_hi, Csplit, reps0, reps1);
}

__global__ __launch_bounds__(256) void gn_bwd_finalize_kernel(const double* __restrict__ gs, const float* __restrict__ mean_rstd,
                                                              const float* __restrict__ gamma, int N, int C, int G,
                                                              double count, int staged, int par, float* __restrict__ dgamma,
                                                              float* __restrict__ dbeta, float* __restrict__ coef,
                                                              const double* __restrict__ gs_hi, int C0, float hi_scale,
                                                              float* __restrict__ coef_hi) {
    extern __shared__ double shb[];
    u3d_gn_bwd_finalize_body(gs, mean_rstd, gamma, N, C, G, count, staged, par, dgamma, dbeta, coef, gs_hi, C0, hi_scale, coef_hi, shb);
}

extern "C" int u3d_gn_bwd_finalize(int device, u3d_stream_t stream, const double* gstats, const float* mean_rstd,
                                   const float* gamma, int N, int C, int G, double count, float* dgamma,
                                   float* dbeta, float* coef) {
    U3D_ENTER(device);
    U3D_REQUIRE(gstats && mean_rstd && gamma && dgamma && dbeta && coef && N > 0 && C > 0 && G > 0 && C % G == 0,
                "u3d_gn_bwd_finalize: bad argument");
    const size_t bytes = sizeof(double) * 2 * (size_t)N * C;
    const int staged = bytes <= 48 * 1024 ? 1 : 0;
    const size_t par_bytes = 2 * bytes + sizeof(double) * 2 * (size_t)N * G;
    const int par = staged && par_bytes <= 64 * 1024 ? 1 : 0;
    hipLaunchKernelGGL(gn_bwd_finalize_kernel, dim3(1), dim3(256), par ? par_bytes : (staged ? bytes : 0), (hipStream_t)stream, gstats,
                       mean_rstd, gamma, N, C, G, count, staged, par, dgamma, dbeta, coef, (const double*)nullptr, C, 1.0f, (float*)nullptr);
    U3D_LAUNCH_CHECK();
    return 0;
}

extern "C" int u3d_gn_bwd_finalize_split_supported(int N, int C, int G) {
    const size_t bytes = sizeof(double) * 2 * (size_t)N * C;
    return (N > 0 && C > 0 && G > 0 && 2 * bytes + sizeof(double) * 2 * (size_t)N * G <= 64 * 1024) ? 1 : 0;
}

extern "C" int u3d_gn_bwd_finalize_split(int device, u3d_stream_t stream, const double* gstats_lo, int C0, const double* gstats_hi,
                                         int C1, const float* mean_rstd, const float* gamma, int N, int G, double count,
                                         float* dgamma, float* dbeta, float* coef, float hi_scale, float* coef_hi) {
    U3D_ENTER(device);
    const int C = C0 + C1;
    U3D_REQUIRE(gstats_lo && gstats_hi && mean_rstd && gamma && dgamma && dbeta && coef && N > 0 && C0 > 0 && C1 > 0 && G > 0 &&
                    C % G == 0, "u3d_gn_bwd_finalize_split: bad argument");
    U3D_REQUIRE(u3d_gn_bwd_finalize_split_supported(N, C, G) == 1, "u3d_gn_bwd_finalize_split: N * C = %d exceeds the staged path", N * C);
    const size_t bytes = sizeof(double) * 2 * (size_t)N * C;
    const size_t par_bytes = 2 * bytes + sizeof(double) * 2 * (size_t)N * G;
    hipLaunchKernelGGL(gn_bwd_finalize_kernel, dim3(1), dim3(256), par_bytes, (hipStream_t)stream, gstats_lo, mean_rstd, gamma, N, C, G,
                       count, 1, 1, dgamma, dbeta, coef, gstats_hi, C0, hi_scale, coef_hi);
    U3D_LAUNCH_CHECK();
    return 0;
}

template <bool VEC, typename T = float>
__global__ void gn_bwd_apply_kernel(const T* __restrict__ dg, int Cdg, int coff, const T* __restrict__ x,
                                    int Cx, const float* __restrict__ coef, int Ctot, long long Vn, int N,
                                    int relu_mask, const T* __restrict__ add, T* __restrict__ out) {
    if (VEC) {
        const int Q = Cx >> 2;
        const long long total = (long long)N * Vn * Q;
        for (long long idx = (long long)blockIdx.x * blockDim.x + threadIdx.x; idx < total;
             idx += (long long)gridDim.x * blockDim.x) {
            const int qd = (int)(idx % Q);
            const long long v = idx / Q;
            const int n = (int)(v / Vn);
            const int c = 4 * qd;
            const f32x4 d = u3d_ldq(dg + (size_t)v * Cdg + coff + c);
            const f32x4 xv = u3d_ldq(x + (size_t)v * Cx + c);
            const f32x4 p = *reinterpret_cast<const f32x4*>(coef + ((size_t)n * 3 + 0) * Ctot + coff + c);
            const f32x4 q = *reinterpret_cast<const f32x4*>(coef + ((size_t)n * 3 + 1) * Ctot + coff + c);
            const f32x4 r = *reinterpret_cast<const f32x4*>(coef + ((size_t)n * 3 + 2) * Ctot + coff + c);
            f32x4 o = p * d + q * xv + r;
            if (add) o += u3d_ldq(add + (size_t)v * Cx + c);
            if (relu_mask) {
#pragma unroll
                for (int e = 0; e < 4; ++e) o[e] = xv[e] > 0.f ? o[e] : 0.f;
            }
            u3d_stq(out + (size_t)v * Cx + c, o);
        }
    } else {
        const long long total = (long long)N * Vn * Cx;
        for (long long idx = (long long)blockIdx.x * blockDim.x + threadIdx.x; idx < total;
             idx += (long long)gridDim.x * blockDim.x) {
            const int c = (int)(idx % Cx);
            const long long v = idx / Cx;
            const int n = (int)(v / Vn);
            const float d = u3d_ld(dg + (size_t)v * Cdg + coff + c);
            const float xv = u3d_ld(x + idx);
            float o = coef[((size_t)n * 3 + 0) * Ctot + coff + c] * d + coef[((size_t)n * 3 + 1) * Ctot + coff + c] * xv +
                      coef[((size_t)n * 3 + 2) * Ctot + coff + c];
            if (add) o += u3d_ld(add + idx);
            if (relu_mask && !(xv > 0.f)) o = 0.f;
            u3d_st(out + idx, o);
        }
    }
}

__global__ __launch_bounds__(256) void gn_bwd_apply_oct_b16_kernel(const __bf16* __restrict__ dg, int Cdg, int coff,
                                                                   const __bf16* __restrict__ x, int Cx, const float* __restrict__ coef,
                                                                   int Ctot, long long Vn, int N, int relu_mask,
                                                                   const __bf16* __restrict__ add, __bf16* __restrict__ out) {
    typedef __bf16 b16x8 __attribute__((ext_vector_type(8)));
    const int Q = Cx >> 3;
    const long long total = (long long)N * Vn * Q;
    for (long long idx = (long long)blockIdx.x * blockDim.x + threadIdx.x; idx < total; idx += (long long)gridDim.x * blockDim.x) {
        const int qd = (int)(idx % Q);
        const long long v = idx / Q;
        const int n = (int)(v / Vn);
        const int c = 8 * qd;
        const b16x8 d8 = *reinterpret_cast<const b16x8*>(dg + (size_t)v * Cdg + coff + c);
        const b16x8 x8 = *reinterpret_cast<const b16x8*>(x + (size_t)v * Cx + c);
        b16x8 a8 = {};
        if (add) a8 = *reinterpret_cast<const b16x8*>(add + (size_t)v * Cx + c);
        const float* cp = coef + ((size_t)n * 3) * Ctot + coff + c;
        b16x8 o8;
#pragma unroll
        for (int hq = 0; hq < 2; ++hq) {
            const f32x4 p = *reinterpret_cast<const f32x4*>(cp + 4 * hq);
            const f32x4 q = *reinterpret_cast<const f32x4*>(cp + Ctot + 4 * hq);
            const f32x4 r = *reinterpret_cast<const f32x4*>(cp + 2 * (size_t)Ctot + 4 * hq);
#pragma unroll
            for (int e = 0; e < 4; ++e) {
                const float xv = (float)x8[4 * hq + e];
                float o = p[e] * (float)d8[4 * hq + e] + q[e] * xv + r[e];
                if (add) o += (float)a8[4 * hq + e];
                if (relu_mask) o = xv > 0.f ? o : 0.f;
                o8[4 * hq + e] = (__bf16)o;
            }
        }
        *reinterpret_cast<b16x8*>(out + (size_t)v * Cx + c) = o8;
    }
}

template <typename T>
static int gn_bwd_apply_impl(int device, u3d_stream_t stream, const T* dg, int Cdg, int coff, const T* x, int Cx,
                             const float* coef, int Ctot, int64_t voxels_per_n, int N, int relu_mask, const T* add,
                             T* out);

extern "C" int u3d_gn_bwd_apply(int device, u3d_stream_t stream, const float* dg, int Cdg, int coff, const float* x,
                                int Cx, const float* coef, int Ctot, int64_t voxels_per_n, int N, int relu_mask,
                                float* out) {
    return gn_bwd_apply_impl<float>(device, stream, dg, Cdg, coff, x, Cx, coef, Ctot, voxels_per_n, N, relu_mask, nullptr, out);
}

extern "C" int u3d_gn_bwd_apply_b16(int device, u3d_stream_t stream, const void* dg, int Cdg, int coff, const void* x, int Cx,
                                    const float* coef, int Ctot, int64_t voxels_per_n, int N, int relu_mask, const void* add,
                                    void* out) {
    return gn_bwd_apply_impl<__bf16>(device, stream, (const __bf16*)dg, Cdg, coff, (const __bf16*)x, Cx, coef, Ctot, voxels_per_n, N,
                                     relu_mask, (const __bf16*)add, (__bf16*)out);
}

extern "C" int u3d_gn_bwd_apply_add(int device, u3d_stream_t stream, const float* dg, int Cdg, int coff, const float* x,
                                    int Cx, const float* coef, int Ctot, int64_t voxels_per_n, int N, int relu_mask,
                                    const float* add, float* out) {
    if (add == nullptr) return u3d_set_err(U3D_EINVAL, "u3d_gn_bwd_apply_add: add is NULL");
    return gn_bwd_apply_impl<float>(device, stream, dg, Cdg, coff, x, Cx, coef, Ctot, voxels_per_n, N, relu_mask, add, out);
}

template <typename T>
static int gn_bwd_apply_impl(int device, u3d_stream_t stream, const T* dg, int Cdg, int coff, const T* x, int Cx,
                             const float* coef, int Ctot, int64_t voxels_per_n, int N, int relu_mask, const T* add,
// ... 1227 lines not shown
```

pytorch-3dunet_amd/pytorch3dunet_amd/_engine_conv.py:

```python
from __future__ import annotations

import copy
import ctypes
import dataclasses
import os
import threading
from dataclasses import dataclass, field
from typing import List, Optional

import torch
import torch.nn.functional as F

from . import _native as nat
from ._native import U3DSrc

from ._engine_base import *
from ._engine_weights import Kind


class _SubLayers(dict):

    plus = frozenset()


@dataclass
class _ConvCall:
    dev: torch.device
    conv: torch.nn.Module
    src: VSrc
    affine: torch.Tensor
    y: torch.Tensor
    N: int
    D: int
    H: int
    W: int
    Ctot: int
    Cout: int
    relu: int
    stats: bool
    pool: _StatPool
    residual: Optional[torch.Tensor]
    sub: dict
    b16: bool
    affine_lo: Optional[torch.Tensor] = None
    affine_hi: Optional[torch.Tensor] = None

    def take_stats(self, reps: int = 1) -> Optional[StatTable]:
        return self.pool.table(self.N, self.Cout, reps) if self.stats else None

    @property
    def flops(self):
        return 54.0 * self.Ctot * self.Cout * self.N * self.D * self.H * self.W


@dataclass
class _BwdCall:
    cx: "_BwdCtx"
    rec: ConvRec
    dz: torch.Tensor
    src: VSrc
    N: int
    D: int
    H: int
    W: int
    Cout: int
    bf16: bool
    b16: bool
    job: object = None
    greps: int = 1

    @property
    def flops(self):
        return 54.0 * self.src.C * self.Cout * self.N * self.D * self.H * self.W


class ConvLayers:

    def _identity_affine(self, N, C, dev):
        key = ("ida", N, C, str(dev))
        t = self._const.get(key)
        if t is None:
            t = self._const[key] = torch.tensor([1.0, 0.0], dtype=_F32, device=dev).repeat(N, C, 1).contiguous()
        return t

    def _identity_coef(self, N, C, dev):
        key = ("idc", N, C, str(dev))
        t = self._const.get(key)
        if t is None:
            t = self._const[key] = torch.tensor([1.0, 0.0, 0.0], dtype=_F32, device=dev).view(1, 3, 1).repeat(N, 1, C).contiguous()
        return t

    def _unact(self, dev, g, y):
        if self.act in (ACT_LEAKY, ACT_ELU):
            nat.call("u3d_act_bwd", dev.index, _stream(dev), _p(g), _p(y), g.numel(), self.act, self.slope, _p(g))

    def _up_scale(self, dev):
        t = getattr(self, "_up_scale_t", None)
        if t is None or t.device != dev:
            t = self._up_scale_t = torch.tensor([1.0, 8.0, 8.0], dtype=_F32, device=dev).view(1, 3, 1)
        return t

    def _subpixel_layers(self, size):
        if not self.subpixel or getattr(self, "is2d", False) or any(ct is not None for ct in self.dec_up) or any(self.dec_interp):
            return _SubLayers()
        dims = [tuple(size)]
        for has_pool, _, _ in self.enc:
            if has_pool:
                dims.append(tuple(d // 2 for d in dims[-1]))
        out, plus = _SubLayers(), set()
        L = len(self.enc)
        for j, (c1, _) in enumerate(self.dec):
            skip_lvl, low_lvl = L - 2 - j, L - 1 - j
            if skip_lvl < 0 or low_lvl >= len(dims) or self._cat_bf16(c1):
                continue
            C0 = self.enc[skip_lvl][2].conv.out_channels
            C1 = c1.conv.in_channels - C0
            ratio = [a - 2 * b for a, b in zip(dims[skip_lvl], dims[low_lvl])]
            if (all(r in (0, 1) for r in ratio) and (self.subpixel_plus or not any(ratio)) and C0 > 0 and C1 > 0 and C0 % 4 == 0
                    and C1 % 4 == 0 and c1.conv.out_channels % 4 == 0):
                out[id(c1.conv.weight)] = (C0, C1)
                if any(ratio):
                    plus.add(id(c1.conv.weight))
        out.plus = frozenset(plus)
        return out

    def _stats_of(self, src: VSrc, st0: Optional[StatTable], st1: Optional[StatTable], pool: _StatPool, dev):
        if src.t1 is None:
            if st0 is None:
                st0 = pool.table(src.N, src.C0, self.stat_reps)
                s = src.struct()
                nat.call("u3d_chan_stats_reps", dev.index, _stream(dev), ctypes.byref(s), src.N, src.D, src.H, src.W, *_tab(st0))
            return st0, None
        if st0 is not None and st1 is not None and src.exact2x and self.fused_stats:
            return st0, dataclasses.replace(st1, scale=8.0)
        plus = src.plus
        if st0 is not None and plus is not None and any(plus) and self.fused_stats and src.C1 % 4 == 0 and src.t1.dtype == _F32:
            st1w = pool.table(src.N, src.C1)
            nat.call("u3d_chan_stats_children", dev.index, _stream(dev), _p(src.t1), src.N, src.D1, src.H1, src.W1, src.C1, *plus,
                     _p(st1w.t))
            return st0, st1w
        st = pool.table(src.N, src.C, self.stat_reps)
        s = src.struct()
        nat.call("u3d_chan_stats_reps", dev.index, _stream(dev), ctypes.byref(s), src.N, src.D, src.H, src.W, *_tab(st))
        return st, None

    def _norm_finalize(self, kind, mod, lo: StatTable, hi: Optional[StatTable], G, count, affine, dev, split=None):
        N, C0, sc0 = lo.N, lo.C, lo.scale
        C1, sc1 = (hi.C, hi.scale) if hi is not None else (0, 0.0)
        if kind == "g" and (lo.reps > 1 or (hi is not None and hi.reps > 1)):
            mean_rstd = _empty((N, G, 2), dtype=_F32, device=dev)
            sp = split if split is not None else (0, None, None)
            p1, r1 = _tab(hi)
# ... 330 lines not shown
        cx, dev, src, rec = c.cx, c.cx.dev, c.src, c.rec
        need = nat.get_lib().u3d_wgrad_bf16_workspace_floats(c.N, c.D, c.H, c.W, src.C, c.Cout)
        ws = cx.ensure_ws(need)
        dw = cx.gview(rec.idx_w)
        job = c.job
        if job is not None and nat.get_lib().u3d_conv3d_wgrad_bf16_job_supported(c.N, c.D, c.H, c.W, src.C, c.Cout, 1 if c.b16 else 0, _p(dw),
                                                                                  job.N, job.C0 + job.C1, job.G) != 1:
            job = None
        nat.call("u3d_conv3d_wgrad_bf16" + ("_b16" if c.b16 else "") + "_job", dev.index, _stream(dev), _p(src.t0), _p(rec.affine), _p(c.dz),
                 _p(dw), c.N, c.D, c.H, c.W, src.C, c.Cout, _p(ws), ws.numel(), ctypes.byref(job) if job is not None else None,
                 flops=c.flops)
        if job is not None:
            c.job = None

    def _wgrad_subpixel(self, c: "_BwdCall"):
        cx, dev, src, rec, ws = c.cx, c.cx.dev, c.src, c.rec, c.cx.ws
        C0, C1 = rec.sub
        Ct = src.C
        dwv = cx.gview(rec.idx_w)
        plus = src.plus
        if any(plus):
            win = (ctypes.c_int * 9)(c.D, c.H, c.W, *plus, *plus)
            nat.call("u3d_subpixel_conv_wgrad_win", dev.index, _stream(dev), _p(src.t1), _p(rec.affine.view(-1)[2 * C0:]), Ct * 2,
                     _p(c.dz), _p(dwv[C0 * 27:]), Ct, c.N, src.D1, src.H1, src.W1, C1, c.Cout, _p(ws), ws.numel(), win,
                     flops=128.0 * C1 * c.Cout * c.N * src.D1 * src.H1 * src.W1)
            s_up = src.up_only_struct(rec.affine_hi if rec.affine_hi is not None else rec.affine[:, C0:].contiguous())
            slice_view = dwv.view(c.Cout, Ct, 27)[:, C0:, :]
            for box in slab_boxes((c.D, c.H, c.W), plus, 2):
                tmp = _empty((c.Cout, C1, 27), dtype=_F32, device=dev)
                nat.call("u3d_conv3d_wgrad_box", dev.index, _stream(dev), ctypes.byref(s_up), _p(c.dz), _p(tmp), c.N, c.D, c.H, c.W,
                         c.Cout, _p(ws), ws.numel(), (ctypes.c_int * 6)(*box),
                         flops=54.0 * C1 * c.Cout * c.N * (box[3] - box[0]) * (box[4] - box[1]) * (box[5] - box[2]))
                slice_view += tmp
        else:
            nat.call("u3d_subpixel_conv_wgrad", dev.index, _stream(dev), _p(src.t1), _p(rec.affine.view(-1)[2 * C0:]), Ct * 2,
                     _p(c.dz), _p(dwv[C0 * 27:]), Ct, c.N, src.D1, src.H1, src.W1, C1, c.Cout, _p(ws), ws.numel(),
                     flops=128.0 * C1 * c.Cout * c.N * src.D1 * src.H1 * src.W1)
        a0 = rec.affine_lo if rec.affine_lo is not None else rec.affine[:, :C0].contiguous()
        s0 = VSrc(src.t0).struct(a0)
        nat.call("u3d_conv3d_wgrad_job", dev.index, _stream(dev), ctypes.byref(s0), _p(c.dz), _p(dwv), Ct, c.N, c.D, c.H, c.W,
                 c.Cout, _p(ws), ws.numel(), ctypes.byref(c.job) if c.job is not None else None,
                 flops=54.0 * C0 * c.Cout * c.N * c.D * c.H * c.W)
        c.job = None

    def _wgrad_fp32_side(self, c: "_BwdCall"):
        cx, dev, src, rec = c.cx, c.cx.dev, c.src, c.rec
        s_aff = src.struct(rec.affine)
        need = nat.get_lib().u3d_wgrad_workspace_floats(c.N, c.D, c.H, c.W, src.C, c.Cout)
        side = cx.side_stream(need)
        side.wait_stream(torch.cuda.current_stream(dev))
        with torch.cuda.stream(side):
            nat.call("u3d_conv3d_wgrad", dev.index, _stream(dev), ctypes.byref(s_aff), _p(c.dz), _p(cx.gview(rec.idx_w)), c.N,
                     c.D, c.H, c.W, c.Cout, _p(cx.ws_side), cx.ws_side.numel(), flops=c.flops)
        c.dz.record_stream(side)
        cx.side_used = True

    def _wgrad_fp32(self, c: "_BwdCall"):
        cx, dev, src, rec, ws = c.cx, c.cx.dev, c.src, c.rec, c.cx.ws
        s_aff = src.struct(rec.affine)
        nat.call("u3d_conv3d_wgrad_job", dev.index, _stream(dev), ctypes.byref(s_aff), _p(c.dz), _p(cx.gview(rec.idx_w)), 0, c.N, c.D,
                 c.H, c.W, c.Cout, _p(ws), ws.numel(), ctypes.byref(c.job) if c.job is not None else None, flops=c.flops)
        c.job = None

    def _dgrad_subpixel(self, c: "_BwdCall"):
        cx, dev, src, rec, ws, pool = c.cx, c.cx.dev, c.src, c.rec, c.cx.ws, c.cx.pool
        Nn, Dd, Hh, Ww, Cout = c.N, c.D, c.H, c.W, c.Cout
        C0, C1 = rec.sub
        w, pair = rec.conv_w, tuple(rec.sub)
        dg0 = _empty((Nn, Dd, Hh, Ww, C0), dtype=_F32, device=dev)
        dlow = _empty_like(src.t1)
        split0 = self._split_dgrad(C0, Cout)
        plus = src.plus
        gst0 = pool.table(Nn, C0, 1 if split0 else c.greps)
        gst1 = pool.table(Nn, C1, 1 if any(plus) else c.greps)
        if split0:
            need = nat.get_lib().u3d_conv3d_bf16_workspace_floats(Nn, Dd, Hh, Ww, Cout, C0)
            kws = cx.ensure_ws(need) if need > 0 else None
            nat.call("u3d_conv3d_f32s", dev.index, _stream(dev), _p(c.dz), None, _p(self.images.get(w, Kind.F32S_DGRAD, dev, pair)),
                     _p(dg0), Nn, Dd, Hh, Ww, Cout, C0, 0, None, _p(src.t0), _p(gst0.t), None, _p(kws), need,
                     flops=54.0 * C0 * Cout * Nn * Dd * Hh * Ww)
        else:
            s_dz = VSrc(c.dz).struct()
            s_x0 = VSrc(src.t0).struct()
            nat.call("u3d_conv3d_ex_reps", dev.index, _stream(dev), ctypes.byref(s_dz), _p(self.images.get(w, Kind.SKIP_DGRAD, dev, pair)), _p(dg0),
                     Nn, Dd, Hh, Ww, C0, 0, None, ctypes.byref(s_x0), _p(gst0.t), None, _p(ws), ws.numel(), gst0.reps,
                     flops=54.0 * C0 * Cout * Nn * Dd * Hh * Ww)
        plus = src.plus
        if any(plus):
            win = (ctypes.c_int * 9)(Dd, Hh, Ww, *plus, *plus)
            nat.call("u3d_subpixel_conv_dgrad_win", dev.index, _stream(dev), _p(c.dz), _p(self.images.get(w, Kind.UP_DGRAD, dev, pair)), _p(src.t1),
                     _p(dlow), _p(gst1.t), Nn, src.D1, src.H1, src.W1, C1, Cout, win,
                     flops=128.0 * C1 * Cout * Nn * src.D1 * src.H1 * src.W1)
            dv = _empty((Nn, Dd, Hh, Ww, C1), dtype=_F32, device=dev)
            s_dz2 = VSrc(c.dz).struct()
            wpd1 = self.images.get(w, Kind.SLAB_DGRAD, dev, pair)
            mask = (ctypes.c_int * 3)(*(2 * e for e in plus))
            for box in slab_boxes((Dd, Hh, Ww), plus, 3):
                nat.call("u3d_conv3d_box", dev.index, _stream(dev), ctypes.byref(s_dz2), _p(wpd1), _p(dv), Nn, Dd, Hh, Ww, C1,
                         (ctypes.c_int * 6)(*box), mask,
                         flops=54.0 * C1 * Cout * Nn * (box[3] - box[0]) * (box[4] - box[1]) * (box[5] - box[2]))
            lz, ly, lx = src.los
            nat.call("u3d_nearest_childsum_add", dev.index, _stream(dev), _p(dv), _p(src.t1), _p(dlow), _p(gst1.t), Nn, Dd, Hh, Ww,
                     src.D1, src.H1, src.W1, C1, _p(lz), _p(ly), _p(lx), *plus)
            del dv
        else:
            nat.call("u3d_subpixel_conv_dgrad_reps", dev.index, _stream(dev), _p(c.dz), _p(self.images.get(w, Kind.UP_DGRAD, dev, pair)), _p(src.t1),
                     _p(dlow), _p(gst1.t), Nn, src.D1, src.H1, src.W1, C1, Cout, gst1.reps,
                     flops=128.0 * C1 * Cout * Nn * src.D1 * src.H1 * src.W1)
        return (dg0, dlow), (gst0, gst1)

    def _dgrad_f32s(self, c: "_BwdCall"):
        cx, dev, src, rec = c.cx, c.cx.dev, c.src, c.rec
        dg = _empty((c.N, c.D, c.H, c.W, src.C), dtype=_F32, device=dev)
        gst = cx.pool.table(c.N, src.C)
        need = nat.get_lib().u3d_conv3d_bf16_workspace_floats(c.N, c.D, c.H, c.W, c.Cout, src.C)
        kws = cx.ensure_ws(need) if need > 0 else None
        nat.call("u3d_conv3d_f32s", dev.index, _stream(dev), _p(c.dz), None, _p(self.images.get(rec.conv_w, Kind.F32S_DGRAD, dev)), _p(dg),
                 c.N, c.D, c.H, c.W, c.Cout, src.C, 0, None, _p(src.t0), _p(gst.t), None, _p(kws), need, flops=c.flops)
        return dg, (gst, None)

    def _dgrad_bf16(self, c: "_BwdCall"):
        cx, dev, src, rec = c.cx, c.cx.dev, c.src, c.rec
        dg = _empty((c.N, c.D, c.H, c.W, src.C), dtype=c.dz.dtype if c.b16 else _F32, device=dev)
        gst = cx.pool.table(c.N, src.C)
        need = nat.get_lib().u3d_conv3d_bf16_workspace_floats(c.N, c.D, c.H, c.W, c.Cout, src.C)
        kws = cx.ensure_ws(need) if need > 0 else None
        nat.call("u3d_conv3d_bf16_ex" + ("_b16" if c.b16 else ""), dev.index, _stream(dev), _p(c.dz), None,
                 _p(self.images.get(rec.conv_w, Kind.BF16_DGRAD, dev)), _p(dg), c.N, c.D, c.H, c.W, c.Cout, src.C, 0, None, _p(src.t0), _p(gst.t),
                 None, _p(kws), need, flops=c.flops)
        return dg, (gst, None)

    def _wgrad_conv2d(self, c: "_BwdCall"):
        cx, dev, src, rec, ws = c.cx, c.cx.dev, c.src, c.rec, c.cx.ws
        s_aff = src.struct(rec.affine)
        nat.call("u3d_conv2d_wgrad", dev.index, _stream(dev), ctypes.byref(s_aff), _p(c.dz), _p(cx.gview(rec.idx_w)), c.N, c.H, c.W,
                 c.Cout, _p(ws), ws.numel(), flops=18.0 * src.C * c.Cout * c.N * c.H * c.W)

    def _dgrad_conv2d(self, c: "_BwdCall"):
        cx, dev, src, rec, ws = c.cx, c.cx.dev, c.src, c.rec, c.cx.ws
        wpd = self.images.get(rec.conv_w, Kind.DGRAD2D, dev)
        dg = _empty((c.N, c.D, c.H, c.W, src.C), dtype=_F32, device=dev)
        gst = cx.pool.table(c.N, src.C, c.greps)
        s_dz = VSrc(c.dz).struct()
        s_x = src.struct()
        nat.call("u3d_conv2d_ex_reps", dev.index, _stream(dev), ctypes.byref(s_dz), _p(wpd), _p(dg), c.N, c.H, c.W, src.C, 0, None,
                 ctypes.byref(s_x), _p(gst.t), _p(ws), ws.numel(), gst.reps, flops=18.0 * src.C * c.Cout * c.N * c.H * c.W)
        return dg, (gst, None)

    def _dgrad_fp32(self, c: "_BwdCall"):
        cx, dev, src, rec, ws = c.cx, c.cx.dev, c.src, c.rec, c.cx.ws
        wpd = self.images.get(rec.conv_w, Kind.DGRAD, dev)
        dg = _empty((c.N, c.D, c.H, c.W, src.C), dtype=_F32, device=dev)
        gst = cx.pool.table(c.N, src.C, c.greps)
        s_dz = VSrc(c.dz).struct()
        s_x = src.struct()
        nat.call("u3d_conv3d_ex_reps", dev.index, _stream(dev), ctypes.byref(s_dz), _p(wpd), _p(dg), c.N, c.D, c.H, c.W, src.C, 0, None,
                 ctypes.byref(s_x), _p(gst.t), None, _p(ws), ws.numel(), gst.reps, flops=c.flops)
        return dg, (gst, None)

    def _conv_bwd(self, cx, rec: ConvRec, dz_, need_dg=True):
        dev, pool, ws, gview = cx.dev, cx.pool, cx.ws, cx.gview
        src = rec.src
        Nn, Dd, Hh, Ww = src.N, src.D, src.H, src.W
        Cout = rec.y.shape[-1]
        if rec.drop is not None:
            kind, mask = rec.drop
            g = _empty_like(dz_)
            if kind == "d":
                nat.call("u3d_mul", dev.index, _stream(dev), _p(dz_), _p(mask), dz_.numel(), _p(g))
            else:
                nat.call("u3d_affine_act_fwd", dev.index, _stream(dev), _p(dz_), _p(mask), Nn, Dd * Hh * Ww, Cout, ACT_NONE, 0.0, _p(g))
            dz_ = g
        if rec.post is not None:
            z, _, inner, islope = rec.post
            Vz = Dd * Hh * Ww
            gst2 = pool.table(Nn, Cout)
            nat.call("u3d_pair_stats", dev.index, _stream(dev), _p(dz_), _p(z), Nn, Vz, Cout, _p(gst2.t))
            if rec.norm is None:
                nat.call("u3d_bias_grad", dev.index, _stream(dev), _p(gst2.t), Nn, Cout, _p(gview(rec.idx_gb)))
            else:
                coef2 = _empty((Nn, 3, Cout), dtype=_F32, device=dev)
                self._norm_bwd_finalize(cx, rec, (gst2, None), float(Vz), coef2)
                dz_ = self._plain_apply(cx, dz_, coef2, z, 1 if inner == ACT_RELU else 0)
                if inner in (ACT_LEAKY, ACT_ELU):
                    nat.call("u3d_act_bwd", dev.index, _stream(dev), _p(dz_), _p(z), dz_.numel(), inner, islope, _p(dz_))
        if self.debug is not None:
            self.debug[rec.name + ".dz"] = dz_.clone()
        if rec.small and not need_dg:
            gst = pool.table(Nn, src.C)
            nat.call("u3d_conv3d_small_cin_bwd", dev.index, _stream(dev), _p(src.t0), _p(rec.affine), _p(dz_),
                     _p(rec.conv_w.detach()), _p(gview(rec.idx_w)), _p(gst.t), Nn, Dd, Hh, Ww, src.C, Cout, _p(ws), ws.numel(),
                     flops=2 * 54.0 * src.C * Cout * Nn * Dd * Hh * Ww)
            if not rec.pre_norm:
                return None, self._identity_coef(Nn, src.C, dev), None
            coef = _empty((Nn, 3, src.C), dtype=_F32, device=dev)
            return None, coef, self._norm_bwd_finalize(cx, rec, (gst, None), float(Dd * Hh * Ww), coef)
        bf16 = src.t1 is None and rec.sub is None and not rec.small and self._bf16_layer(src.C, Cout)
        b16 = src.t0.dtype == torch.bfloat16
        assert not b16 or (bf16 and Cout % 64 == 0 and dz_.dtype == torch.bfloat16)
        call = _BwdCall(cx, rec, dz_, src, Nn, Dd, Hh, Ww, Cout, bf16, b16)
        if (self.stat_reps > 1 and rec.pre_norm and rec.norm == "g" and self._wgrad_family(call) in ("fp32", "subpixel")
                and nat.get_lib().u3d_conv3d_wgrad_job_supported(Nn, src.C, rec.G) == 1):
            call.greps = self.stat_reps
        dg, gst = getattr(self, self._DGRAD_KERNELS[self._dgrad_family(call)])(call)
        if self.debug is not None and rec.sub is None:
            self.debug[rec.name + ".dg"] = dg.clone()
        coef = coef_hi = None
        if rec.pre_norm:
            coef = _empty((Nn, 3, src.C), dtype=_F32, device=dev)
            call.job, coef_hi = self._norm_bwd_job(cx, rec, gst, float(Dd * Hh * Ww), coef)
        had_job = call.job is not None
        getattr(self, self._WGRAD_KERNELS[self._wgrad_family(call)])(call)
        if not rec.pre_norm:
            return dg, self._identity_coef(Nn, src.C, dev), None
        if not had_job or call.job is not None:
            coef_hi = self._norm_bwd_finalize(cx, rec, gst, float(Dd * Hh * Ww), coef)
        return dg, coef, coef_hi

    def _plain_apply(self, cx, dg, coef, x, relu_mask, add=None):
        dev = cx.dev
        out = _empty_like(x)
        Nn = x.shape[0]
        C = x.shape[-1]
        if x.dtype == torch.bfloat16:
            nat.call("u3d_gn_bwd_apply_b16", dev.index, _stream(dev), _p(dg), C, 0, _p(x), C, _p(coef), C, x.numel() // (Nn * C), Nn,
                     relu_mask, _p(add), _p(out))
            return out
        if add is None:
            nat.call("u3d_gn_bwd_apply", dev.index, _stream(dev), _p(dg), C, 0, _p(x), C, _p(coef), C, x.numel() // (Nn * C), Nn,
                     relu_mask, _p(out))
        else:
            nat.call("u3d_gn_bwd_apply_add", dev.index, _stream(dev), _p(dg), C, 0, _p(x), C, _p(coef), C,
                     x.numel() // (Nn * C), Nn, relu_mask, _p(add), _p(out))
        return out

    def _wgrad_workspace(self, tape, dev):
        return _empty(max(self._wgrad_workspace_floats(tape.convs), 4), dtype=_F32, device=dev)

    def _layer_ws_floats(self, N, D, H, W, Cin, Cout, sub=None, small=False, virtual=False):
        lib = nat.get_lib()
        if getattr(self, "is2d", False):
            return max(lib.u3d_wgrad2d_workspace_floats(N, H, W, Cin, Cout), lib.u3d_conv2d_workspace_floats(N, H, W, Cout, Cin))
        if small:
            return lib.u3d_small_cin_bwd_workspace_floats(N, D, H, W, Cin, Cout)
        if sub is not None:
            boxes = slab_boxes((D, H, W), (D % 2, H % 2, W % 2), 2)
            return max([lib.u3d_wgrad_workspace_floats(N, D, H, W, sub[0], Cout),
                        lib.u3d_subpixel_wgrad_workspace_floats(N, D // 2, H // 2, W // 2, sub[1], Cout),
                        lib.u3d_conv3d_workspace_floats(N, D, H, W, Cout, sub[0])] +
                       [lib.u3d_wgrad_workspace_floats(N, b[3] - b[0], b[4] - b[1], b[5] - b[2], sub[1], Cout) for b in boxes])
        if not virtual and self._bf16_layer(Cin, Cout):
            need = lib.u3d_conv3d_bf16_workspace_floats(N, D, H, W, Cout, Cin)
            wg = lib.u3d_wgrad_bf16_workspace_floats(N, D, H, W, Cin, Cout)
            return max(need, wg)
        return max(lib.u3d_wgrad_workspace_floats(N, D, H, W, Cin, Cout), lib.u3d_conv3d_workspace_floats(N, D, H, W, Cout, Cin))

    def _wgrad_workspace_floats(self, convs):
        need = 0
        for r in convs:
            need = max(need, self._layer_ws_floats(r.src.N, r.src.D, r.src.H, r.src.W, r.src.C, r.y.shape[-1], r.sub, r.small,
                                                   r.src.t1 is not None))
        return int(need)
```

pytorch-3dunet_amd/pytorch3dunet_amd/_engine_unet.py:

```python
from __future__ import annotations

import copy
import ctypes
import dataclasses
import os
import threading
from dataclasses import dataclass, field
from typing import List, Optional

import torch
import torch.nn.functional as F

from . import _native as nat
from ._native import U3DSrc

from ._engine_base import *
from ._engine_conv import ConvLayers
from ._engine_weights import Kind, WeightImages



class UNet3DEngine(ConvLayers):

    def __init__(self, model):
# ... 177 lines not shown
                _, Ds, Hs, Ws, _ = sk.shape
                tabs = [_resample_tables(dev, self.dec_interp[j], a, b) for a, b in ((D1, Ds), (H1, Hs), (W1, Ws))]
                up = _empty((Nl, Ds, Hs, Ws, Cl), dtype=_F32, device=dev)
                nat.call("u3d_resample2_fwd", dev.index, _stream(dev), _p(cur), _p(tabs[0][0]), _p(tabs[1][0]), _p(tabs[2][0]),
                         _p(tabs[0][1]), _p(tabs[1][1]), _p(tabs[2][1]), Nl, D1, H1, W1, Ds, Hs, Ws, Cl, _p(up))
                if tape is not None:
                    tape.ups.append(UpRec(cur, None, tabs, (Ds, Hs, Ws)))
                cur, cur_st = up, None
            src = VSrc(sk, cur)
            st_in = stats_of(src, sk_st, cur_st, pool, dev)
            if self._cat_bf16(c1):
                cat = _empty((src.N, src.D, src.H, src.W, src.C), dtype=_F32, device=dev)
                nat.call("u3d_nearest_cat_fwd", dev.index, _stream(dev), _p(sk), _p(cur), _p(src.maps[0]), _p(src.maps[1]), _p(src.maps[2]),
                         src.N, src.D, src.H, src.W, src.D1, src.H1, src.W1, src.C0, src.C1, _p(cat))
                if tape is not None:
                    tape.cats[j] = src
                y1, s1 = self._single_conv_fwd(c1, f"dec{j}.c1", VSrc(cat), st_in, pool, tape)
                del cat
            else:
                y1, s1 = self._single_conv_fwd(c1, f"dec{j}.c1", src, st_in, pool, tape, sub=sub)
            src2 = VSrc(y1)
            y2, s2 = self._single_conv_fwd(c2, f"dec{j}.c2", src2, stats_of(src2, s1, None, pool, dev), pool, tape)
            cur, cur_st = y2, s2

        fc = m.final_conv
        Co, Cf = fc.out_channels, fc.in_channels
        V = D * H * W
        logits = _empty((N, Co, D, H, W), dtype=_F32, device=dev)
        act = 0
        probs = None
        if m.final_activation is not None:
            act = 1 if isinstance(m.final_activation, torch.nn.Sigmoid) else 2
            probs = _empty_like(logits)
        nat.call("u3d_conv1x1_head_fwd", dev.index, _stream(dev), _p(cur), _p(fc.weight.detach()), _p(fc.bias.detach()), N, V,
                 Cf, Co, act, _p(logits), _p(probs))
        if tape is not None:
            tape.head_x = cur
            if self.debug is not None:
                self.debug["tape"] = tape
        if self.is2d:
            logits = logits.view(N, Co, H, W)
            probs = probs.view(N, Co, H, W) if probs is not None else None
        return logits, probs, tape

    def backward(self, tape: Tape, dlogits: torch.Tensor, need_input_grad: bool):
        m = self.model
        dev = dlogits.device
        N, Cin, D, H, W = tape.dims
        V = D * H * W
        dlogits = dlogits.contiguous()
        flat = _empty(self.n_params, dtype=_F32, device=dev)

        def gview(idx):
            p = self.params[idx]
            return flat[self.poffs[idx] : self.poffs[idx] + p.numel()]

        fc = m.final_conv
        Co, Cf = fc.out_channels, fc.in_channels
        tot = self.stat_reps * (Co * Cf + Co) + sum(self.stat_reps * N * r.src.C * 2 for r in tape.convs)
        pool = getattr(tape, "bwd_pool", None)
        tape.bwd_pool = None
        if (pool is None or pool.buf.numel() < tot or pool.buf.device != dev or torch.cuda.is_current_stream_capturing()
                or not pool.claim()):
            pool = _StatPool(dev, tot)
        ws = self._wgrad_workspace(tape, dev)

        hreps = self.stat_reps
        hacc = pool.take(hreps * (Co * Cf + Co))
        dz = _empty_like(tape.head_x)
        nat.call("u3d_conv1x1_head_bwd_reps", dev.index, _stream(dev), _p(dlogits), _p(tape.head_x), _p(fc.weight.detach()), N, V,
                 Cf, Co, self.mask, _p(dz), _p(hacc), hreps)
        self._unact(dev, dz, tape.head_x)
        iw, ib = self._pindex[id(fc.weight)], self._pindex[id(fc.bias)]
        assert self.poffs[ib] == self.poffs[iw] + Co * Cf
        nat.call("u3d_cvt_f64_f32_sum", dev.index, _stream(dev), _p(hacc), _p(gview(iw)), Co * Cf + Co, hreps)

        n_levels = len(self.enc)
        n_dec = len(self.dec)
        mk = self.mask
        skip_grad = {}

        cx = _BwdCtx(dev, pool, ws, flat, self)

        def conv_bwd(rec: ConvRec, dz_, need_dg=True):
            return self._conv_bwd(cx, rec, dz_, need_dg)

        def plain_apply(dg, coef, x, relu_mask):
            return self._plain_apply(cx, dg, coef, x, relu_mask)

        recs = tape.convs
        enc_recs = [(recs[2 * i], recs[2 * i + 1]) for i in range(n_levels)]
        dec_recs = [(recs[2 * n_levels + 2 * j], recs[2 * n_levels + 2 * j + 1]) for j in range(n_dec)]

        for j in range(n_dec - 1, -1, -1):
            r1, r2 = dec_recs[j]
            dg2, coef2, _ = conv_bwd(r2, dz)
            dz1 = plain_apply(dg2, coef2, r2.src.t0, mk)
            self._unact(dev, dz1, r2.src.t0)
            del dg2
            dg1, coef1, coef_hi = conv_bwd(r1, dz1)
            src = tape.cats.get(j, r1.src)
            C0, C1, Ct = src.C0, src.C1, src.C
            lvl = n_levels - 2 - j
            dzl = _empty_like(src.t1)
            if r1.sub is not None:
                dg0, dlow = dg1
                skip_grad[lvl] = (dg0, C0, coef1, Ct)
                if any(src.plus):
                    nat.call("u3d_gn_bwd_apply_children", dev.index, _stream(dev), _p(dlow), _p(src.t1), _p(coef1), Ct, C0, src.N, src.D1,
                             src.H1, src.W1, C1, *src.plus, mk, _p(dzl))
                else:
                    coef_up = coef_hi if coef_hi is not None else coef1[:, :, C0:] * self._up_scale(dev)
                    nat.call("u3d_gn_bwd_apply", dev.index, _stream(dev), _p(dlow), C1, 0, _p(src.t1), C1, _p(coef_up), C1,
                             src.D1 * src.H1 * src.W1, src.N, mk, _p(dzl))
                del dg0, dlow
            else:
                skip_grad[lvl] = (dg1, Ct, coef1, Ct)
                lz, ly, lx = src.los
                nat.call("u3d_gn_bwd_apply_up", dev.index, _stream(dev), _p(dg1), Ct, C0, _p(src.t1), C1, _p(coef1), Ct, src.N,
                         src.D, src.H, src.W, src.D1, src.H1, src.W1, _p(lz), _p(ly), _p(lx),
                         0 if (self.dec_up[j] is not None or self.dec_interp[j] is not None) else mk, _p(dzl))
            del dg1
            if self.dec_up[j] is not None:
                up = tape.ups[j]
                xl = up.x_low
                Nl, D1, H1, W1, Cl = xl.shape
                Cs = up.weight.shape[1]
                acc = pool.take(up.weight.numel())
                dxl = _empty_like(xl)
                nat.call("u3d_convtr3d_bwd", dev.index, _stream(dev), _p(dzl), _p(xl), _p(up.weight.detach()), Nl, D1, H1, W1, Cl, Cs,
                         mk, _p(dxl), _p(acc), _p(self.images.get(up.weight, Kind.CONVTR_DGRAD, dev)), flops=4.0 * 27 * Cl * Cs * Nl * D1 * H1 * W1)
                nat.call("u3d_cvt_f64_f32", dev.index, _stream(dev), _p(acc), _p(gview(self._pindex[id(up.weight)])),
                         up.weight.numel())
                self._unact(dev, dxl, xl)
                dzl = dxl
            elif self.dec_interp[j] is not None:
                up = tape.ups[j]
                xl = up.x_low
                Nl, D1, H1, W1, Cl = xl.shape
                Ds, Hs, Ws = up.tdims
                tz, ty, tx = up.los
                dxl = _empty_like(xl)
                nat.call("u3d_resample2_bwd", dev.index, _stream(dev), _p(dzl), _p(tz[2]), _p(ty[2]), _p(tx[2]), _p(tz[0]), _p(ty[0]),
                         _p(tx[0]), _p(tz[1]), _p(ty[1]), _p(tx[1]), Nl, D1, H1, W1, Ds, Hs, Ws, Cl, _p(dxl))
                if self.act != ACT_NONE:
                    nat.call("u3d_act_bwd", dev.index, _stream(dev), _p(dxl), _p(xl), dxl.numel(), self.act, self.slope, _p(dxl))
                dzl = dxl
            else:
                self._unact(dev, dzl, src.t1)
            dz = dzl

        if self.grad_sync is not None:
            cx.join()
            self.grad_sync.launch(flat[self.n_enc_params :])

        dx0 = None
        pending_hi = self.n_enc_params
        for i in range(n_levels - 1, -1, -1):
            r1, r2 = enc_recs[i]
            dg2, coef2, _ = conv_bwd(r2, dz)
            dz1 = plain_apply(dg2, coef2, r2.src.t0, mk)
            self._unact(dev, dz1, r2.src.t0)
            del dg2
            dg1, coef1, _ = conv_bwd(r1, dz1, need_dg=(i > 0 or need_input_grad))
            if self.grad_sync is not None:
                pending_hi = self._sync_encoder_level(cx, flat, i, pending_hi)
            if i > 0:
                pooled, argmax, e_in = tape.pools[i - 1]
                Ne, De, He, We, Ce = e_in.shape
                out = _empty_like(e_in)
                sk = skip_grad.pop(i - 1, None)
                pdims = (Ne, He, We, Ce) if self.is2d else (Ne, De, He, We, Ce)
                sfx = "2d" if self.is2d else "2"
                if sk is None:
                    nat.call(f"u3d_maxpool{sfx}_bwd_merge", dev.index, _stream(dev), _p(dg1), _p(pooled), _p(argmax), _p(coef1), None,
                             _p(e_in), *pdims, mk, _p(out))
                else:
                    sdg, sCdg, scoef, sCt = sk
                    nat.call(f"u3d_maxpool{sfx}_bwd_merge_gn", dev.index, _stream(dev), _p(dg1), _p(pooled), _p(argmax), _p(coef1),
                             _p(sdg), sCdg, _p(scoef), sCt, _p(e_in), *pdims, mk, _p(out))
                    del sk, sdg, scoef
                self._unact(dev, out, e_in)
                dz = out
            elif need_input_grad:
                dx0 = plain_apply(dg1, coef1, tape.x0, 0)
            del dg1

        cx.join()
        if self.grad_sync is not None:
            self.grad_sync.finish()

        dx = None
        if dx0 is not None:
            if Cin == 1:
                dx = dx0.view(N, 1, D, H, W)
            else:
                dx = _empty((N, Cin, D, H, W), dtype=_F32, device=dev)
                nat.call("u3d_ndhwc_to_ncdhw", dev.index, _stream(dev), _p(dx0), _p(dx), N, Cin, V)
            if self.is2d:
                dx = dx.view(N, Cin, H, W)
        return flat, dx
```

pytorch-3dunet_amd/pytorch3dunet_amd/_native.py:

```python
from __future__ import annotations

import ctypes
import os
import threading
from ctypes import POINTER, c_char_p, c_double, c_float, c_int, c_int32, c_int64, c_size_t, c_void_p

_HERE = os.path.dirname(os.path.abspath(__file__))
LIB_PATH = os.environ.get("U3D_LIB_PATH") or os.path.join(_HERE, "lib", "libu3d_hip.so")

U3D_OK = 0


class U3DSrc(ctypes.Structure):

    _fields_ = [
        ("p0", c_void_p),
        ("p1", c_void_p),
        ("zmap", c_void_p),
        ("ymap", c_void_p),
        ("xmap", c_void_p),
        ("affine", c_void_p),
        ("C0", c_int32),
        ("C1", c_int32),
        ("D1", c_int32),
# ... 47 lines not shown
    ),
    "u3d_conv3d_small_cin_fwd": (
        c_int,
        [c_int, c_void_p, c_void_p, c_void_p, c_void_p, c_void_p, c_int, c_int, c_int, c_int, c_int, c_int, c_int, c_void_p],
    ),
    "u3d_conv3d_small_cin_fwd_reps": (
        c_int,
        [c_int, c_void_p, c_void_p, c_void_p, c_void_p, c_void_p, c_int, c_int, c_int, c_int, c_int, c_int, c_int, c_void_p, c_int],
    ),
    "u3d_small_cin_bwd_workspace_floats": (c_size_t, [c_int, c_int, c_int, c_int, c_int, c_int]),
    "u3d_conv3d_small_cin_bwd": (
        c_int,
        [c_int, c_void_p, c_void_p, c_void_p, c_void_p, c_void_p, c_void_p, c_void_p, c_int, c_int, c_int, c_int, c_int,
         c_int, c_void_p, c_size_t],
    ),
    "u3d_conv3d_naive": (
        c_int,
        [c_int, c_void_p, POINTER(U3DSrc), c_void_p, c_void_p, c_int, c_int, c_int, c_int, c_int, c_int, c_int, c_int],
    ),
    "u3d_chan_stats": (c_int, [c_int, c_void_p, POINTER(U3DSrc), c_int, c_int, c_int, c_int, c_void_p]),
    "u3d_chan_stats_reps": (c_int, [c_int, c_void_p, POINTER(U3DSrc), c_int, c_int, c_int, c_int, c_void_p, c_int]),
    "u3d_gn_finalize": (
        c_int,
        [c_int, c_void_p, c_void_p, c_int, c_double, c_void_p, c_int, c_double, c_int, c_int, c_double, c_void_p,
         c_void_p, c_float, c_void_p, c_void_p],
    ),
    "u3d_gn_bwd_finalize": (
        c_int,
        [c_int, c_void_p, c_void_p, c_void_p, c_void_p, c_int, c_int, c_int, c_double, c_void_p, c_void_p, c_void_p],
    ),
    "u3d_gn_finalize_split": (
        c_int,
        [c_int, c_void_p, c_void_p, c_int, c_double, c_void_p, c_int, c_double, c_int, c_int, c_double, c_void_p,
         c_void_p, c_float, c_void_p, c_void_p, c_int, c_void_p, c_void_p],
    ),
    "u3d_gn_bwd_finalize_split_supported": (c_int, [c_int, c_int, c_int]),
    "u3d_chan_stats_children": (c_int, [c_int, c_void_p, c_void_p, c_int, c_int, c_int, c_int, c_int, c_int, c_int, c_int, c_void_p]),
    "u3d_adam_step": (c_int, [c_int, c_void_p, c_void_p, c_int, c_int64, c_double, c_double, c_double, c_double, c_double, c_int64]),
    "u3d_gn_bwd_finalize_split": (
        c_int,
        [c_int, c_void_p, c_void_p, c_int, c_void_p, c_int, c_void_p, c_void_p, c_int, c_int, c_double, c_void_p, c_void_p,
         c_void_p, c_float, c_void_p],
    ),
    "u3d_gn_bwd_apply": (
        c_int,
        [c_int, c_void_p, c_void_p, c_int, c_int, c_void_p, c_int, c_void_p, c_int, c_int64, c_int, c_int, c_void_p],
    ),
    "u3d_gn_bwd_apply_up": (
        c_int,
        [c_int, c_void_p, c_void_p, c_int, c_int, c_void_p, c_int, c_void_p, c_int, c_int, c_int, c_int, c_int, c_int,
         c_int, c_int, c_void_p, c_void_p, c_void_p, c_int, c_void_p],
    ),
    "u3d_maxpool2_fwd": (c_int, [c_int, c_void_p, c_void_p, c_int, c_int, c_int, c_int, c_int, c_void_p, c_void_p, c_void_p]),
    "u3d_maxpool2_bwd_merge": (
        c_int,
        [c_int, c_void_p, c_void_p, c_void_p, c_void_p, c_void_p, c_void_p, c_void_p, c_int, c_int, c_int, c_int, c_int,
         c_int, c_void_p],
    ),
    "u3d_maxpool2_bwd_merge_gn": (
        c_int,
        [c_int, c_void_p, c_void_p, c_void_p, c_void_p, c_void_p, c_void_p, c_int, c_void_p, c_int, c_void_p, c_int, c_int,
         c_int, c_int, c_int, c_int, c_void_p],
    ),
    "u3d_conv1x1_head_fwd": (
        c_int,
        [c_int, c_void_p, c_void_p, c_void_p, c_void_p, c_int, c_int64, c_int, c_int, c_int, c_void_p, c_void_p],
    ),
    "u3d_conv1x1_head_bwd": (
        c_int,
        [c_int, c_void_p, c_void_p, c_void_p, c_void_p, c_int, c_int64, c_int, c_int, c_int, c_void_p, c_void_p],
    ),
    "u3d_conv1x1_head_bwd_reps": (
        c_int,
        [c_int, c_void_p, c_void_p, c_void_p, c_void_p, c_int, c_int64, c_int, c_int, c_int, c_void_p, c_void_p, c_int],
    ),
    "u3d_conv3d_wgrad_strided": (
        c_int,
        [c_int, c_void_p, POINTER(U3DSrc), c_void_p, c_void_p, c_int, c_int, c_int, c_int, c_int, c_int, c_void_p, c_size_t],
    ),
    "u3d_conv3d_ex_reps": (
        c_int,
        [c_int, c_void_p, POINTER(U3DSrc), c_void_p, c_void_p, c_int, c_int, c_int, c_int, c_int, c_int, c_void_p, POINTER(U3DSrc),
         c_void_p, c_void_p, c_void_p, c_int64, c_int],
    ),
    "u3d_gn_finalize_reps": (
        c_int,
        [c_int, c_void_p, c_void_p, c_int, c_double, c_int, c_void_p, c_int, c_double, c_int, c_int, c_int, c_double, c_void_p, c_void_p,
         c_float, c_void_p, c_void_p, c_int, c_void_p, c_void_p],
    ),
    "u3d_conv3d_wgrad_job_supported": (c_int, [c_int, c_int, c_int]),
    "u3d_conv3d_wgrad_job": (
        c_int,
        [c_int, c_void_p, POINTER(U3DSrc), c_void_p, c_void_p, c_int, c_int, c_int, c_int, c_int, c_int, c_void_p, c_size_t,
         POINTER(U3DGnBwdJob)],
    ),
    "u3d_subpixel_wgrad_workspace_floats": (c_int64, [c_int, c_int, c_int, c_int, c_int, c_int]),
    "u3d_subpixel_conv_wgrad": (
        c_int,
        [c_int, c_void_p, c_void_p, c_void_p, c_int64, c_void_p, c_void_p, c_int, c_int, c_int, c_int, c_int, c_int, c_int,
         c_void_p, c_int64],
    ),
    "u3d_convtr3d_subpixel_packed_floats": (c_int64, [c_int, c_int]),
    "u3d_pack_convtr3d_subpixel": (c_int, [c_int, c_void_p, c_void_p, c_int, c_int, c_void_p]),
    "u3d_convtr3d_fwd_subpixel": (
        c_int, [c_int, c_void_p, c_void_p, c_void_p, c_void_p, c_int, c_int, c_int, c_int, c_int, c_int],
    ),
    "u3d_subpixel_packed_floats": (c_int64, [c_int, c_int]),
    "u3d_subpixel_dgrad_packed_floats": (c_int64, [c_int, c_int]),
    "u3d_pack_subpixel_dgrad_weights": (c_int, [c_int, c_void_p, c_void_p, c_int, c_int, c_int, c_int, c_void_p]),
    "u3d_subpixel_conv_dgrad": (
        c_int,
        [c_int, c_void_p, c_void_p, c_void_p, c_void_p, c_void_p, c_void_p, c_int, c_int, c_int, c_int, c_int, c_int],
    ),
    "u3d_subpixel_conv_dgrad_reps": (
        c_int,
        [c_int, c_void_p, c_void_p, c_void_p, c_void_p, c_void_p, c_void_p, c_int, c_int, c_int, c_int, c_int, c_int, c_int],
    ),
    "u3d_pack_subpixel_weights": (c_int, [c_int, c_void_p, c_void_p, c_int, c_int, c_int, c_int, c_void_p]),
    "u3d_subpixel_conv_fwd_win": (c_int, [c_int, c_void_p, c_void_p, c_void_p, c_int64, c_void_p, c_void_p, c_int, c_int, c_int, c_int,
                                          c_int, c_int, POINTER(c_int)]),
    "u3d_subpixel_conv_dgrad_win": (c_int, [c_int, c_void_p, c_void_p, c_void_p, c_void_p, c_void_p, c_void_p, c_int, c_int, c_int, c_int,
                                            c_int, c_int, POINTER(c_int)]),
    "u3d_subpixel_conv_wgrad_win": (c_int, [c_int, c_void_p, c_void_p, c_void_p, c_int64, c_void_p, c_void_p, c_int, c_int, c_int, c_int,
                                            c_int, c_int, c_int, c_void_p, c_int64, POINTER(c_int)]),
    "u3d_conv3d_box": (c_int, [c_int, c_void_p, POINTER(U3DSrc), c_void_p, c_void_p, c_int, c_int, c_int, c_int, c_int, POINTER(c_int),
                               POINTER(c_int)]),
    "u3d_conv3d_wgrad_box": (c_int, [c_int, c_void_p, POINTER(U3DSrc), c_void_p, c_void_p, c_int, c_int, c_int, c_int, c_int, c_void_p,
                                     c_size_t, POINTER(c_int)]),
    "u3d_gn_bwd_apply_children": (c_int, [c_int, c_void_p, c_void_p, c_void_p, c_void_p, c_int, c_int, c_int, c_int, c_int, c_int, c_int,
                                          c_int, c_int, c_int, c_int, c_void_p]),
    "u3d_nearest_childsum_add": (c_int, [c_int, c_void_p, c_void_p, c_void_p, c_void_p, c_void_p, c_int, c_int, c_int, c_int, c_int, c_int,
                                         c_int, c_int, c_void_p, c_void_p, c_void_p, c_int, c_int, c_int]),
    "u3d_subpixel_fwd_workspace_floats": (c_int64, [c_int, c_int, c_int, c_int, c_int, c_int]),
    "u3d_subpixel_conv_fwd": (
        c_int,
        [c_int, c_void_p, c_void_p, c_void_p, c_int64, c_void_p, c_void_p, c_int, c_int, c_int, c_int, c_int, c_int,
         c_void_p, c_int64],
    ),
    "u3d_conv3d_workspace_floats": (c_int64, [c_int, c_int, c_int, c_int, c_int, c_int]),
    "u3d_conv3d_ex": (
        c_int,
        [c_int, c_void_p, POINTER(U3DSrc), c_void_p, c_void_p, c_int, c_int, c_int, c_int, c_int, c_int, c_void_p,
         POINTER(U3DSrc), c_void_p, c_void_p, c_void_p, c_int64],
    ),
    "u3d_conv3d_residual": (
        c_int,
        [c_int, c_void_p, POINTER(U3DSrc), c_void_p, c_void_p, c_int, c_int, c_int, c_int, c_int, c_int, c_void_p, c_void_p],
    ),
    "u3d_gn_bwd_apply_add": (
        c_int,
        [c_int, c_void_p, c_void_p, c_int, c_int, c_void_p, c_int, c_void_p, c_int, c_int64, c_int, c_int, c_void_p, c_void_p],
    ),
    "u3d_conv1x1_fwd": (c_int, [c_int, c_void_p, c_void_p, c_void_p, c_void_p, c_void_p, c_int, c_int64, c_int, c_int, c_void_p]),
    "u3d_conv1x1_bwd": (c_int, [c_int, c_void_p, c_void_p, c_void_p, c_void_p, c_int, c_int64, c_int, c_int, c_void_p, c_void_p]),
    "u3d_pack_convtr_weights": (c_int, [c_int, c_void_p, c_void_p, c_int, c_int, c_int, c_void_p]),
    "u3d_convtr3d_fwd": (c_int, [c_int, c_void_p, c_void_p, c_void_p, c_void_p, c_int, c_int, c_int, c_int, c_int, c_int, c_void_p]),
    "u3d_convtr3d_bwd": (
        c_int,
        [c_int, c_void_p, c_void_p, c_void_p, c_void_p, c_int, c_int, c_int, c_int, c_int, c_int, c_int, c_void_p, c_void_p,
         c_void_p],
    ),
    "u3d_nearest_add_fwd": (
        c_int,
        [c_int, c_void_p, c_void_p, c_void_p, c_void_p, c_void_p, c_void_p, c_int, c_int, c_int, c_int, c_int, c_int, c_int,
         c_int, c_void_p, c_void_p],
    ),
# ... 332 lines not shown
```

Measured before the change: 121.0.

## Fuse GroupNorm backward apply into conv dgrad halo staging

```diff
diff --git a/include/u3d.h b/include/u3d.h
--- a/include/u3d.h
+++ b/include/u3d.h
@@ -65,6 +65,11 @@
 int u3d_conv3d_ex_reps(int device, u3d_stream_t stream, const u3d_src_t* src, const float* packed_w, float* out, int N,
                        int D, int H, int W, int Cout, int relu, double* out_stats, const u3d_src_t* gx, double* gstats,
                        const float* residual, float* workspace, long long workspace_floats, int stat_reps);
+
+int u3d_conv3d_dgrad_gnbwd_supported(int N, int D, int H, int W, int Cin, int Cout);
+int u3d_conv3d_dgrad_gnbwd_reps(int device, u3d_stream_t stream, const float* dg, const float* x, const float* coef, int relu_mask,
+                                float* dz_out, int Cin, const float* packed_w, float* out, int N, int D, int H, int W, int Cout,
+                                const u3d_src_t* gx, double* gstats, int stat_reps);
 
 long long u3d_subpixel_packed_floats(int C1, int Cout);
 long long u3d_subpixel_dgrad_packed_floats(int Cout, int C1);
diff --git a/pytorch-3dunet_amd/csrc/u3d_conv.hip b/pytorch-3dunet_amd/csrc/u3d_conv.hip
--- a/pytorch-3dunet_amd/csrc/u3d_conv.hip
+++ b/pytorch-3dunet_amd/csrc/u3d_conv.hip
@@ -5,7 +5,7 @@
 #include "u3d_gn.h"
 #include "u3d_subpix.h"
 
-int g_u3d_tune[24] = {0};
+int g_u3d_tune[25] = {0};
 
 namespace cv {
 constexpr int TZ = 4, TY = 8, TX = 8;
@@ -51,6 +51,10 @@
     long long* dbg;
     int oz0, oy0, ox0, oz1, oy1, ox1;
     int mz, my, mx;
+    const float* gnb_x;
+    const float* gnb_coef;
+    float* gnb_dz;
+    int gnb_relu;
 };
 
 #define U3D_DBG_STAMP(slot)                                                   \
@@ -530,13 +534,14 @@
     if constexpr (E > B) u3d_for_rows_impl<B>(std::make_integer_sequence<int, E - B>{}, static_cast<F&&>(f));
 }
 
-template <int NT, bool VIRT, bool DBG = false, bool PAIRY = false, bool AFF = true, bool N16 = false, bool RAG = false>
+template <int NT, bool VIRT, bool DBG = false, bool PAIRY = false, bool AFF = true, bool N16 = false, bool RAG = false, bool GNB = false>
 __global__ __launch_bounds__(256, 2) void conv3d_mfma_reg_kernel(const ConvParams p) {
     using namespace cv;
+    static_assert(!GNB || (!VIRT && !DBG && !PAIRY && !AFF && !N16 && !RAG && NT == 1), "staged-source mode: plain source, aligned volume, NT = 1");
     static_assert(!RAG || (!PAIRY && !DBG), "ragged tiles: standard and 16-column variants only");
     static_assert(!PAIRY || NT == 1, "the paired-y variant has a single N-tile");
     static_assert(!N16 || (NT == 1 && !PAIRY), "the 16-column variant has a single N-tile");
-    constexpr int RB = NT == 1 ? 9 : 3;
+    constexpr int RB = NT == 1 ? (GNB ? 6 : 9) : 3;
     constexpr int MT = N16 ? 4 : (PAIRY ? 1 : 2);
     constexpr int RY = PAIRY ? 4 : 3;
     constexpr int NROWS = 3 * RY;
@@ -579,6 +584,7 @@
     const int q = t & 3, tv = t >> 2;
     int rel0[NIT], rel1[VIRT ? NIT : 1], loff[NIT];
     unsigned fz0 = 0, fz1 = 0, fy0 = 0, fy1 = 0, fx0 = 0, fx1 = 0, fdead = 0;
+    unsigned fint = 0;
     const int vz = RAG && D % TZ ? D % TZ : TZ, vy = RAG && H % TY ? H % TY : TY, vx = RAG && W % TX ? W % TX : TX;
 #pragma unroll
     for (int it = 0; it < NIT; ++it) {
@@ -598,6 +604,7 @@
         fx0 |= (in && hx == 0 ? 1u : 0u) << it;
         fx1 |= (in && hx > vx ? 1u : 0u) << it;
         fdead |= (in ? 0u : 1u) << it;
+        if constexpr (GNB) fint |= (in && hz >= 1 && hz <= TZ && hy >= 1 && hy <= TY && hx >= 1 && hx <= TX ? 1u : 0u) << it;
     }
     struct Digits {
         int cb, xi, yi, zi, n;
@@ -690,6 +697,9 @@
         bool cok, from0;
         const float* ap;
         f32x4 lo, hi;
+        int gofs;
+        const float* cp;
+        f32x4 gp, gq, gr;
     };
     auto chunk_src = [&](int ch, int n, bool live) {
         ChunkSrc c;
@@ -701,6 +711,11 @@
         c.ap = p.src.affine ? p.src.affine + ((size_t)n * Ctot + (c.cok ? cq : 0)) * 2 : nullptr;
         c.lo = f32x4{1.f, 0.f, 1.f, 0.f};
         c.hi = f32x4{1.f, 0.f, 1.f, 0.f};
+        if constexpr (GNB) {
+            c.gofs = c.cok ? cq : 0;
+            c.cp = p.gnb_coef + (size_t)n * 3 * Ctot;
+            c.gp = c.gq = c.gr = f32x4{0.f, 0.f, 0.f, 0.f};
+        }
         return c;
     };
     auto load_affine_rows = [&](ChunkSrc& c) {
@@ -711,13 +726,29 @@
             }
         }
     };
+    auto load_coef_rows = [&](ChunkSrc& c) {
+        c.gp = *reinterpret_cast<const f32x4*>(c.cp + c.gofs);
+        c.gq = *reinterpret_cast<const f32x4*>(c.cp + Ctot + c.gofs);
+        c.gr = *reinterpret_cast<const f32x4*>(c.cp + 2 * Ctot + c.gofs);
+    };
     auto halo_load = [&](const ChunkSrc& c, const Item& S, int it, bool masked) {
         int idx = c.from0 ? S.base0 + rel0[it] : S.base1 + rel1[VIRT ? it : 0];
         if (masked) idx = (c.cok && ((S.inv >> it) & 1u) == 0) ? idx : 0;
         return *reinterpret_cast<const f32x4*>(c.base + (size_t)idx * c.Cs);
     };
-    auto halo_store = [&](float* buf, const ChunkSrc& c, const Item& S, int it, f32x4 raw, bool masked) {
+    auto halo_load_x = [&](const ChunkSrc& c, const Item& S, int it, bool masked) {
+        int idx = S.base0 + rel0[it];
+        if (masked) idx = (c.cok && ((S.inv >> it) & 1u) == 0) ? idx : 0;
+        return *reinterpret_cast<const f32x4*>(p.gnb_x + ((size_t)idx * Ctot + c.gofs));
+    };
+    auto halo_store = [&](float* buf, const ChunkSrc& c, const Item& S, int it, f32x4 raw, bool masked, f32x4 xraw = f32x4{0.f, 0.f, 0.f, 0.f},
+                          bool formed = false) {
         f32x4 val = raw;
+        if constexpr (GNB) {
+            if (!formed) val = u3d_gn_bwd_dz(raw, xraw, c.gp, c.gq, c.gr, nullptr, p.gnb_relu);
+            if (S.cb == 0 && ((fint >> it) & 1u) != 0 && (!masked || c.cok))
+                *reinterpret_cast<f32x4*>(p.gnb_dz + ((size_t)(S.base0 + rel0[it]) * Ctot + c.gofs)) = val;
+        }
         if constexpr (AFF)
             val = f32x4{fmaf(raw[0], c.lo[0], c.lo[1]), fmaf(raw[1], c.lo[2], c.lo[3]), fmaf(raw[2], c.hi[0], c.hi[1]),
                         fmaf(raw[3], c.hi[2], c.hi[3])};
@@ -759,12 +790,21 @@
     {
         ChunkSrc c0 = chunk_src(0, T.n, true);
         load_affine_rows(c0);
+        if constexpr (GNB) load_coef_rows(c0);
         const bool masked = T.border || dead_quads || fdead != 0;
         f32x4 v[NIT];
 #pragma unroll
         for (int it = 0; it < NIT; ++it) v[it] = halo_load(c0, T, it, true);
-#pragma unroll
-        for (int it = 0; it < NIT; ++it) halo_store(lds, c0, T, it, v[it], true);
+        if constexpr (GNB) {
+            f32x4 xv[NIT];
+#pragma unroll
+            for (int it = 0; it < NIT; ++it) xv[it] = halo_load_x(c0, T, it, true);
+#pragma unroll
+            for (int it = 0; it < NIT; ++it) halo_store(lds, c0, T, it, v[it], true, xv[it]);
+        } else {
+#pragma unroll
+            for (int it = 0; it < NIT; ++it) halo_store(lds, c0, T, it, v[it], true);
+        }
         (void)masked;
     }
     u3d_flag_signal(&cnt[0], l);
@@ -811,6 +851,9 @@
             ChunkSrc cn = chunk_src(nch_, S.n, has_next);
             const bool masked = S.border || !has_next || (dead_quads && nch_ + 1 == p.nchunks);
             f32x4 v[NIT];
+            constexpr int NIH = NIT / 2;
+            static_assert(NIT % 2 == 0, "the x quads are loaded in two halves");
+            f32x4 xv[GNB ? NIH : 1];
             u3d_flag_wait(&cnt[b], 4 * (gch / 2 + 1));
             __builtin_amdgcn_s_setprio(0);
             if (ntiles == DBG_TILE && ch < 7) U3D_DBG_STAMP(8 + 2 * ch);
@@ -820,7 +863,7 @@
 #pragma unroll
             for (int mt = 0; mt < MT; ++mt) aq[0][mt] = *reinterpret_cast<const f32x4*>(&cur[abase + mrow(mt) * RS]);
             const f32x4* wch0 = wq + (size_t)(ch * NSTEPL + RB - 1) * wstep;
-            enum { ROW_PLAIN = 0, ROW_LOAD = 1, ROW_AFFINE = 2, ROW_STORE = 3, ROW_LAST = 4, ROW_LOAD_FIRST = 5 };
+            enum { ROW_PLAIN = 0, ROW_LOAD = 1, ROW_AFFINE = 2, ROW_STORE = 3, ROW_LAST = 4, ROW_LOAD_FIRST = 5, ROW_GX0 = 6, ROW_GX1 = 7 };
             auto row_body = [&](auto kind_c, auto row_c) __attribute__((always_inline)) {
                 constexpr int KIND = decltype(kind_c)::value;
                 constexpr int row = decltype(row_c)::value;
@@ -830,6 +873,7 @@
                 const float* anext = cur + abase + (nrow / RY) * PS + (nrow % RY) * RS;
                 const bool do_store = KIND == ROW_STORE && has_next;
                 if constexpr (KIND == ROW_AFFINE) load_affine_rows(cn);
+                if constexpr (KIND == ROW_GX0) load_coef_rows(cn);
                 if constexpr (KIND == ROW_STORE) {
                     if (do_store) u3d_flag_wait(&cnt[2 + (b ^ 1)], 4 * ((gch + 1) / 2));
                 }
@@ -850,6 +894,22 @@
                             } else {
 #pragma unroll
                                 for (int it = 0; it < NIT; ++it) v[it] = halo_load(cn, S, it, false);
+                            }
+                        }
+                    }
+                    if constexpr (KIND == ROW_GX0 || KIND == ROW_GX1) {
+                        if (s6 == 0) {
+                            constexpr int I0 = KIND == ROW_GX0 ? 0 : NIH;
+                            if constexpr (KIND == ROW_GX1) {
+#pragma unroll
+                                for (int it = 0; it < NIH; ++it) v[it] = u3d_gn_bwd_dz(v[it], xv[it], cn.gp, cn.gq, cn.gr, nullptr, p.gnb_relu);
+                            }
+                            if (masked) {
+#pragma unroll
+                                for (int it = 0; it < NIH; ++it) xv[it] = halo_load_x(cn, S, I0 + it, true);
+                            } else {
+#pragma unroll
+                                for (int it = 0; it < NIH; ++it) xv[it] = halo_load_x(cn, S, I0 + it, false);
                             }
                         }
                     }
@@ -891,9 +951,9 @@
                                 const int it = s6 * STORES_PER_STEP + k;
                                 if (it < NIT) {
                                     if (masked)
-                                        halo_store(nxt, cn, S, it, v[it], true);
+                                        halo_store(nxt, cn, S, it, v[it], true, xv[GNB ? it % NIH : 0], it < NIH);
                                     else
-                                        halo_store(nxt, cn, S, it, v[it], false);
+                                        halo_store(nxt, cn, S, it, v[it], false, xv[GNB ? it % NIH : 0], it < NIH);
                                 }
                             }
                             if ((s6 + 1) * STORES_PER_STEP >= NIT) u3d_flag_signal(&cnt[b ^ 1], l);
@@ -925,7 +985,14 @@
                 row_body(std::integral_constant<int, ROW_LOAD_FIRST>{}, R0{});
             else
                 row_body(std::integral_constant<int, ROW_LOAD>{}, R0{});
-            u3d_for_rows<1, ISTORE - 1>([&](auto r) { row_body(std::integral_constant<int, ROW_PLAIN>{}, r); });
+            if constexpr (GNB) {
+                static_assert(ISTORE == 5, "rows 2 and 3 load the x halves, row 5 stores");
+                row_body(std::integral_constant<int, ROW_PLAIN>{}, std::integral_constant<int, 1>{});
+                row_body(std::integral_constant<int, ROW_GX0>{}, std::integral_constant<int, 2>{});
+                row_body(std::integral_constant<int, ROW_GX1>{}, std::integral_constant<int, 3>{});
+            } else {
+                u3d_for_rows<1, ISTORE - 1>([&](auto r) { row_body(std::integral_constant<int, ROW_PLAIN>{}, r); });
+            }
             row_body(std::integral_constant<int, ROW_AFFINE>{}, std::integral_constant<int, ISTORE - 1>{});
             row_body(std::integral_constant<int, ROW_STORE>{}, std::integral_constant<int, ISTORE>{});
             u3d_for_rows<ISTORE + 1, NROWS - 1>([&](auto r) { row_body(std::integral_constant<int, ROW_PLAIN>{}, r); });
@@ -1885,7 +1952,7 @@
 }
 
 extern "C" int u3d_set_tuning(int key, int value) {
-    if (key < 0 || key >= 24) return u3d_set_err(U3D_EINVAL, "u3d_set_tuning: key out of range");
+    if (key < 0 || key >= 25) return u3d_set_err(U3D_EINVAL, "u3d_set_tuning: key out of range");
     g_u3d_tune[key] = value;
     return 0;
 }
@@ -1968,6 +2035,9 @@
                                 hipFuncAttributeMaxDynamicSharedMemorySize, bytes));
     U3D_HIP(hipFuncSetAttribute(reinterpret_cast<const void*>(conv3d_mfma_reg_kernel<NT, false, false, false, true, false, true>),
                                 hipFuncAttributeMaxDynamicSharedMemorySize, bytes));
+    if constexpr (NT == 1)
+        U3D_HIP(hipFuncSetAttribute(reinterpret_cast<const void*>(conv3d_mfma_reg_kernel<NT, false, false, false, false, false, false, true>),
+                                    hipFuncAttributeMaxDynamicSharedMemorySize, bytes));
     if (NT == 1) {
         U3D_HIP(hipFuncSetAttribute(reinterpret_cast<const void*>(conv3d_mfma_reg_kernel<1, true, false, false, true, true, true>),
                                     hipFuncAttributeMaxDynamicSharedMemorySize, bytes));
@@ -2017,10 +2087,17 @@
     return 0;
 }
 
+struct GnbArgs {
+    const float* x;
+    const float* coef;
+    float* dz_out;
+    int relu_mask;
+};
+
 static int conv3d_impl(int device, u3d_stream_t stream, const u3d_src_t* src, const float* packed_w, float* out, int N,
                        int D, int H, int W, int Cout, int relu, double* out_stats, const u3d_src_t* gx, double* gstats,
                        const float* residual, float* ws = nullptr, long long ws_floats = 0, const int* out_box = nullptr,
-                       const int* in_mask = nullptr, int stat_reps = 1);
+                       const int* in_mask = nullptr, int stat_reps = 1, const GnbArgs* gnb = nullptr);
 
 extern "C" int u3d_conv3d(int device, u3d_stream_t stream, const u3d_src_t* src, const float* packed_w, float* out,
                           int N, int D, int H, int W, int Cout, int relu, double* out_stats, const u3d_src_t* gx,
@@ -2060,6 +2137,41 @@
     return (long long)ks * N * D * H * W * Cout;
 }
 
+static int conv_ntiles_per_block(long long ntiles, int ntot) {
+    int nt = 1;
+    if (ntot % 3 == 0 && ntiles * (ntot / 3) >= 512) nt = 3;
+    else if (ntot % 2 == 0 && ntiles * (ntot / 2) >= 512) nt = 2;
+    if (g_u3d_tune[0] >= 1 && g_u3d_tune[0] <= 3 && ntot % g_u3d_tune[0] == 0) nt = g_u3d_tune[0];
+    return nt;
+}
+
+extern "C" int u3d_conv3d_dgrad_gnbwd_supported(int N, int D, int H, int W, int Cin, int Cout) {
+    if (N <= 0 || D <= 0 || H <= 0 || W <= 0 || Cin <= 0 || Cout <= 0) return 0;
+    if (g_u3d_tune[24] == 1 || g_u3d_tune[3] != 0) return 0;
+    if (Cin % 4 != 0 || Cout % 4 != 0 || Cout <= 16) return 0;
+    if (D % cv::TZ != 0 || H % cv::TY != 0 || W % cv::TX != 0) return 0;
+    if ((long long)N * D * H * W >= (1ll << 31)) return 0;
+    if (splitk_shape(N, D, H, W, Cin, Cout)) return 0;
+    const long long ntiles = (long long)N * (D / cv::TZ) * (H / cv::TY) * (W / cv::TX);
+    return conv_ntiles_per_block(ntiles, cdiv(Cout, 32)) == 1 ? 1 : 0;
+}
+
+extern "C" int u3d_conv3d_dgrad_gnbwd_reps(int device, u3d_stream_t stream, const float* dg, const float* x, const float* coef,
+                                           int relu_mask, float* dz_out, int Cin, const float* packed_w, float* out, int N, int D, int H,
+                                           int W, int Cout, const u3d_src_t* gx, double* gstats, int stat_reps) {
+    U3D_REQUIRE(dg && x && coef && dz_out, "u3d_conv3d_dgrad_gnbwd_reps: bad argument");
+    U3D_REQUIRE(u3d_conv3d_dgrad_gnbwd_supported(N, D, H, W, Cin, Cout) == 1,
+                "u3d_conv3d_dgrad_gnbwd_reps: shape outside the fused kernel (ask u3d_conv3d_dgrad_gnbwd_supported)");
+    U3D_REQUIRE((((uintptr_t)dg | (uintptr_t)x | (uintptr_t)coef | (uintptr_t)dz_out | (uintptr_t)out) & 15) == 0,
+                "u3d_conv3d_dgrad_gnbwd_reps: tensors must be 16-byte aligned");
+    U3D_REQUIRE(!gx || (gx->C1 == 0 && src_vec_ok(gx)), "u3d_conv3d_dgrad_gnbwd_reps: gx must be a plain tensor readable in channel quads");
+    u3d_src_t s = {};
+    s.p0 = dg, s.C0 = Cin;
+    const GnbArgs g = {x, coef, dz_out, relu_mask};
+    return conv3d_impl(device, stream, &s, packed_w, out, N, D, H, W, Cout, 0, nullptr, gx, gstats, nullptr, nullptr, 0, nullptr, nullptr,
+                       stat_reps, &g);
+}
+
 extern "C" int u3d_conv3d_ex(int device, u3d_stream_t stream, const u3d_src_t* src, const float* packed_w, float* out,
                              int N, int D, int H, int W, int Cout, int relu, double* out_stats, const u3d_src_t* gx,
                              double* gstats, const float* residual, float* workspace, long long workspace_floats) {
@@ -2085,7 +2197,8 @@
 
 static int conv3d_impl(int device, u3d_stream_t stream, const u3d_src_t* src, const float* packed_w, float* out, int N,
                        int D, int H, int W, int Cout, int relu, double* out_stats, const u3d_src_t* gx, double* gstats,
-                       const float* residual, float* ws, long long ws_floats, const int* out_box, const int* in_mask, int stat_reps) {
+                       const float* residual, float* ws, long long ws_floats, const int* out_box, const int* in_mask, int stat_reps,
+                       const GnbArgs* gnb) {
     U3D_ENTER(device);
     if (int e = check_src(src, "u3d_conv3d")) return e;
     U3D_REQUIRE(stat_reps >= 1 && stat_reps <= 64, "u3d_conv3d: stat_reps must be 1 .. 64");
@@ -2130,11 +2243,10 @@
     p.ovec = (Cout % 4 == 0 && ((uintptr_t)out & 15) == 0 && (!gx || src_vec_ok(gx)) &&
               (!residual || ((uintptr_t)residual & 15) == 0)) ? 1 : 0;
     const long long ntiles = (long long)N * p.tz * p.ty * p.tx;
-    int nt = 1;
-    if (p.ntot % 3 == 0 && ntiles * (p.ntot / 3) >= 512) nt = 3;
-    else if (p.ntot % 2 == 0 && ntiles * (p.ntot / 2) >= 512) nt = 2;
-    if (g_u3d_tune[0] >= 1 && g_u3d_tune[0] <= 3 && p.ntot % g_u3d_tune[0] == 0) nt = g_u3d_tune[0];
+    const int nt = conv_ntiles_per_block(ntiles, p.ntot);
     p.ncb = p.ntot / nt;
+    p.gnb_x = gnb ? gnb->x : nullptr, p.gnb_coef = gnb ? gnb->coef : nullptr, p.gnb_dz = gnb ? gnb->dz_out : nullptr;
+    p.gnb_relu = gnb ? gnb->relu_mask : 0;
     const long long nblk = ntiles * p.ncb;
     U3D_REQUIRE(nblk < (1ll << 31), "u3d_conv3d: grid too large");
     const size_t shmem = cv::LDS_FLOATS * sizeof(float);
@@ -2195,6 +2307,13 @@
         const bool virt = p.src.C1 > 0;
         const bool noaff = p.src.affine == nullptr && g_u3d_tune[7] == 0;
         p.dbg = (!ragged && g_u3d_prof_buf && (size_t)slots * 4 <= g_u3d_prof_records) ? g_u3d_prof_buf : nullptr;
+        if (gnb) {
+            U3D_REQUIRE(!ragged && !virt && nt == 1 && p.src.affine == nullptr, "u3d_conv3d_dgrad_gnbwd_reps: launcher and query disagree");
+            p.dbg = nullptr;
+            hipLaunchKernelGGL((conv3d_mfma_reg_kernel<1, false, false, false, false, false, false, true>), rgrid, rblock, shmem, st, p);
+            U3D_LAUNCH_CHECK();
+            return 0;
+        }
         if (ragged) {
             if (Cout <= 16 && nt == 1 && p.ntot == 1) {
                 p.wp = packed_w + ((size_t)p.nchunks * cv::NSTEP + cv::PACK_PAD) * 256 + ((size_t)p.nchunks * cv::NSTEP_PAIRY + cv::PACK_PAD) * 256;
@@ -2272,6 +2391,7 @@
         U3D_LAUNCH_CHECK();
         return 0;
     }
+    U3D_REQUIRE(!gnb, "u3d_conv3d_dgrad_gnbwd_reps: launcher and query disagree");
     const bool vec = p.vec != 0;
     const dim3 grid((unsigned)nblk), block(256);
     p.dbg = (vec && g_u3d_prof_buf && (size_t)nblk * 4 <= g_u3d_prof_records) ? g_u3d_prof_buf : nullptr;
diff --git a/pytorch-3dunet_amd/csrc/u3d_gn.h b/pytorch-3dunet_amd/csrc/u3d_gn.h
--- a/pytorch-3dunet_amd/csrc/u3d_gn.h
+++ b/pytorch-3dunet_amd/csrc/u3d_gn.h
@@ -11,6 +11,19 @@
         for (int j = 0; j < 8; ++j) v += t[j];
     }
     return v;
+}
+
+__device__ __forceinline__ f32x4 u3d_gn_bwd_dz(f32x4 d, f32x4 xv, f32x4 p, f32x4 q, f32x4 r, const f32x4* add, int relu_mask) {
+#pragma clang fp contract(off)
+    const f32x4 t = q * xv;
+    f32x4 o = __builtin_elementwise_fma(p, d, t);
+    o = o + r;
+    if (add) o = o + *add;
+    if (relu_mask) {
+#pragma unroll
+        for (int e = 0; e < 4; ++e) o[e] = xv[e] > 0.f ? o[e] : 0.f;
+    }
+    return o;
 }
 
 __device__ inline void u3d_gn_bwd_finalize_body(const double* __restrict__ gs, const float* __restrict__ mean_rstd,
diff --git a/pytorch-3dunet_amd/csrc/u3d_ops.hip b/pytorch-3dunet_amd/csrc/u3d_ops.hip
--- a/pytorch-3dunet_amd/csrc/u3d_ops.hip
+++ b/pytorch-3dunet_amd/csrc/u3d_ops.hip
@@ -494,13 +494,9 @@
             const f32x4 p = *reinterpret_cast<const f32x4*>(coef + ((size_t)n * 3 + 0) * Ctot + coff + c);
             const f32x4 q = *reinterpret_cast<const f32x4*>(coef + ((size_t)n * 3 + 1) * Ctot + coff + c);
             const f32x4 r = *reinterpret_cast<const f32x4*>(coef + ((size_t)n * 3 + 2) * Ctot + coff + c);
-            f32x4 o = p * d + q * xv + r;
-            if (add) o += u3d_ldq(add + (size_t)v * Cx + c);
-            if (relu_mask) {
-#pragma unroll
-                for (int e = 0; e < 4; ++e) o[e] = xv[e] > 0.f ? o[e] : 0.f;
-            }
-            u3d_stq(out + (size_t)v * Cx + c, o);
+            f32x4 av;
+            if (add) av = u3d_ldq(add + (size_t)v * Cx + c);
+            u3d_stq(out + (size_t)v * Cx + c, u3d_gn_bwd_dz(d, xv, p, q, r, add ? &av : nullptr, relu_mask));
         }
     } else {
         const long long total = (long long)N * Vn * Cx;
diff --git a/pytorch-3dunet_amd/pytorch3dunet_amd/_engine_conv.py b/pytorch-3dunet_amd/pytorch3dunet_amd/_engine_conv.py
--- a/pytorch-3dunet_amd/pytorch3dunet_amd/_engine_conv.py
+++ b/pytorch-3dunet_amd/pytorch3dunet_amd/_engine_conv.py
@@ -68,6 +68,7 @@
     b16: bool
     job: object = None
     greps: int = 1
+    fuse: Optional[tuple] = None
 
     @property
     def flops(self):
@@ -564,9 +565,15 @@
         else:
             s_dz = VSrc(c.dz).struct()
             s_x0 = VSrc(src.t0).struct()
-            nat.call("u3d_conv3d_ex_reps", dev.index, _stream(dev), ctypes.byref(s_dz), _p(self.images.get(w, Kind.SKIP_DGRAD, dev, pair)), _p(dg0),
-                     Nn, Dd, Hh, Ww, C0, 0, None, ctypes.byref(s_x0), _p(gst0.t), None, _p(ws), ws.numel(), gst0.reps,
-                     flops=54.0 * C0 * Cout * Nn * Dd * Hh * Ww)
+            if c.fuse is not None:
+                fdg, fx, fcoef, fmask = c.fuse
+                nat.call("u3d_conv3d_dgrad_gnbwd_reps", dev.index, _stream(dev), _p(fdg), _p(fx), _p(fcoef), fmask, _p(c.dz), Cout,
+                         _p(self.images.get(w, Kind.SKIP_DGRAD, dev, pair)), _p(dg0), Nn, Dd, Hh, Ww, C0, ctypes.byref(s_x0), _p(gst0.t),
+                         gst0.reps, flops=54.0 * C0 * Cout * Nn * Dd * Hh * Ww)
+            else:
+                nat.call("u3d_conv3d_ex_reps", dev.index, _stream(dev), ctypes.byref(s_dz), _p(self.images.get(w, Kind.SKIP_DGRAD, dev, pair)),
+                         _p(dg0), Nn, Dd, Hh, Ww, C0, 0, None, ctypes.byref(s_x0), _p(gst0.t), None, _p(ws), ws.numel(), gst0.reps,
+                         flops=54.0 * C0 * Cout * Nn * Dd * Hh * Ww)
         plus = src.plus
         if any(plus):
             win = (ctypes.c_int * 9)(Dd, Hh, Ww, *plus, *plus)
@@ -636,11 +643,34 @@
         gst = cx.pool.table(c.N, src.C, c.greps)
         s_dz = VSrc(c.dz).struct()
         s_x = src.struct()
+        if c.fuse is not None:
+            fdg, fx, fcoef, fmask = c.fuse
+            nat.call("u3d_conv3d_dgrad_gnbwd_reps", dev.index, _stream(dev), _p(fdg), _p(fx), _p(fcoef), fmask, _p(c.dz), c.Cout, _p(wpd),
+                     _p(dg), c.N, c.D, c.H, c.W, src.C, ctypes.byref(s_x), _p(gst.t), gst.reps, flops=c.flops)
+            return dg, (gst, None)
         nat.call("u3d_conv3d_ex_reps", dev.index, _stream(dev), ctypes.byref(s_dz), _p(wpd), _p(dg), c.N, c.D, c.H, c.W, src.C, 0, None,
                  ctypes.byref(s_x), _p(gst.t), None, _p(ws), ws.numel(), gst.reps, flops=c.flops)
         return dg, (gst, None)
 
-    def _conv_bwd(self, cx, rec: ConvRec, dz_, need_dg=True):
+    def _fuse_gn_bwd(self, rec: ConvRec, dg, coef, x, relu_mask, need_dg=True):
+        src = rec.src
+        Cout = rec.y.shape[-1]
+        if (not need_dg or getattr(self, "is2d", False) or x.dtype != _F32 or dg.dtype != _F32 or rec.drop is not None
+                or rec.post is not None or rec.small or self.act in (ACT_LEAKY, ACT_ELU)):
+            return None
+        if rec.sub is not None:
+            Cd = rec.sub[0]
+        elif src.t1 is None and not self._bf16_layer(src.C, Cout):
+            Cd = src.C
+        else:
+            return None
+        if self._split_dgrad(Cd, Cout):
+            return None
+        if nat.get_lib().u3d_conv3d_dgrad_gnbwd_supported(src.N, src.D, src.H, src.W, Cout, Cd) != 1:
+            return None
+        return (dg, x, coef, relu_mask)
+
+    def _conv_bwd(self, cx, rec: ConvRec, dz_, need_dg=True, fuse=None):
         dev, pool, ws, gview = cx.dev, cx.pool, cx.ws, cx.gview
         src = rec.src
         Nn, Dd, Hh, Ww = src.N, src.D, src.H, src.W
@@ -666,7 +696,7 @@
                 dz_ = self._plain_apply(cx, dz_, coef2, z, 1 if inner == ACT_RELU else 0)
                 if inner in (ACT_LEAKY, ACT_ELU):
                     nat.call("u3d_act_bwd", dev.index, _stream(dev), _p(dz_), _p(z), dz_.numel(), inner, islope, _p(dz_))
-        if self.debug is not None:
+        if self.debug is not None and fuse is None:
             self.debug[rec.name + ".dz"] = dz_.clone()
         if rec.small and not need_dg:
             gst = pool.table(Nn, src.C)
@@ -680,11 +710,14 @@
         bf16 = src.t1 is None and rec.sub is None and not rec.small and self._bf16_layer(src.C, Cout)
         b16 = src.t0.dtype == torch.bfloat16
         assert not b16 or (bf16 and Cout % 64 == 0 and dz_.dtype == torch.bfloat16)
-        call = _BwdCall(cx, rec, dz_, src, Nn, Dd, Hh, Ww, Cout, bf16, b16)
+        call = _BwdCall(cx, rec, dz_, src, Nn, Dd, Hh, Ww, Cout, bf16, b16, fuse=fuse)
+        assert fuse is None or self._dgrad_family(call) in ("fp32", "subpixel")
         if (self.stat_reps > 1 and rec.pre_norm and rec.norm == "g" and self._wgrad_family(call) in ("fp32", "subpixel")
                 and nat.get_lib().u3d_conv3d_wgrad_job_supported(Nn, src.C, rec.G) == 1):
             call.greps = self.stat_reps
         dg, gst = getattr(self, self._DGRAD_KERNELS[self._dgrad_family(call)])(call)
+        if self.debug is not None and fuse is not None:
+            self.debug[rec.name + ".dz"] = dz_.clone()
         if self.debug is not None and rec.sub is None:
             self.debug[rec.name + ".dg"] = dg.clone()
         coef = coef_hi = None
diff --git a/pytorch-3dunet_amd/pytorch3dunet_amd/_engine_unet.py b/pytorch-3dunet_amd/pytorch3dunet_amd/_engine_unet.py
--- a/pytorch-3dunet_amd/pytorch3dunet_amd/_engine_unet.py
+++ b/pytorch-3dunet_amd/pytorch3dunet_amd/_engine_unet.py
@@ -283,8 +283,16 @@
 
         cx = _BwdCtx(dev, pool, ws, flat, self)
 
-        def conv_bwd(rec: ConvRec, dz_, need_dg=True):
-            return self._conv_bwd(cx, rec, dz_, need_dg)
+        def conv_bwd(rec: ConvRec, dz_, need_dg=True, fuse=None):
+            return self._conv_bwd(cx, rec, dz_, need_dg, fuse)
+
+        def mid_dz(rec1, dg2, coef2, x, need_dg=True):
+            fuse = self._fuse_gn_bwd(rec1, dg2, coef2, x, mk, need_dg)
+            if fuse is not None:
+                return _empty_like(x), fuse
+            dz1 = plain_apply(dg2, coef2, x, mk)
+            self._unact(dev, dz1, x)
+            return dz1, None
 
         def plain_apply(dg, coef, x, relu_mask):
             return self._plain_apply(cx, dg, coef, x, relu_mask)
@@ -296,10 +304,10 @@
         for j in range(n_dec - 1, -1, -1):
             r1, r2 = dec_recs[j]
             dg2, coef2, _ = conv_bwd(r2, dz)
-            dz1 = plain_apply(dg2, coef2, r2.src.t0, mk)
-            self._unact(dev, dz1, r2.src.t0)
+            dz1, fuse = mid_dz(r1, dg2, coef2, r2.src.t0)
             del dg2
-            dg1, coef1, coef_hi = conv_bwd(r1, dz1)
+            dg1, coef1, coef_hi = conv_bwd(r1, dz1, fuse=fuse)
+            del fuse
             src = tape.cats.get(j, r1.src)
             C0, C1, Ct = src.C0, src.C1, src.C
             lvl = n_levels - 2 - j
@@ -360,10 +368,11 @@
         for i in range(n_levels - 1, -1, -1):
             r1, r2 = enc_recs[i]
             dg2, coef2, _ = conv_bwd(r2, dz)
-            dz1 = plain_apply(dg2, coef2, r2.src.t0, mk)
-            self._unact(dev, dz1, r2.src.t0)
+            need_dg1 = i > 0 or need_input_grad
+            dz1, fuse = mid_dz(r1, dg2, coef2, r2.src.t0, need_dg1)
             del dg2
-            dg1, coef1, _ = conv_bwd(r1, dz1, need_dg=(i > 0 or need_input_grad))
+            dg1, coef1, _ = conv_bwd(r1, dz1, need_dg=need_dg1, fuse=fuse)
+            del fuse
             if self.grad_sync is not None:
                 pending_hi = self._sync_encoder_level(cx, flat, i, pending_hi)
             if i > 0:
diff --git a/pytorch-3dunet_amd/pytorch3dunet_amd/_native.py b/pytorch-3dunet_amd/pytorch3dunet_amd/_native.py
--- a/pytorch-3dunet_amd/pytorch3dunet_amd/_native.py
+++ b/pytorch-3dunet_amd/pytorch3dunet_amd/_native.py
@@ -153,6 +153,12 @@
         c_int,
         [c_int, c_void_p, POINTER(U3DSrc), c_void_p, c_void_p, c_int, c_int, c_int, c_int, c_int, c_int, c_void_p, POINTER(U3DSrc),
          c_void_p, c_void_p, c_void_p, c_int64, c_int],
+    ),
+    "u3d_conv3d_dgrad_gnbwd_supported": (c_int, [c_int, c_int, c_int, c_int, c_int, c_int]),
+    "u3d_conv3d_dgrad_gnbwd_reps": (
+        c_int,
+        [c_int, c_void_p, c_void_p, c_void_p, c_void_p, c_int, c_void_p, c_int, c_void_p, c_void_p, c_int, c_int, c_int, c_int, c_int,
+         POINTER(U3DSrc), c_void_p, c_int],
     ),
     "u3d_gn_finalize_reps": (
         c_int,
```

Result: no change. 121.4, median of 6 (+0.4%).
